# tgialoimtr/cnn_lstm_ctc_ocr

Hardware: AMD Instinct MI355X
Metric: line-crops/sec (train step) at 32x256 bs=256; CER vs ref (higher is better)
Workload: dtype bf16

## Files before the change

### cnn_lstm_ctc_ocr_amd/_lib.py

```python
import ctypes
import os

import torch

_HERE = os.path.dirname(os.path.abspath(__file__))
LIB_PATH = os.environ.get("OCRK_LIB") or os.path.join(_HERE, "libocrk.so")

OCRK_OK = 0
OCRK_ERR_INVALID_ARG = 1
OCRK_ERR_HIP = 2
OCRK_ERR_INFEASIBLE = 3

F32 = 0
BF16 = 1

_p = ctypes.c_void_p
_i32 = ctypes.c_int
_u32 = ctypes.c_uint
_i64 = ctypes.c_int64
_f32 = ctypes.c_float
_sz = ctypes.c_size_t

SIGNATURES = {
    "ocrk_version": [],
# ... 5 lines not shown
    "ocrk_set_f32_gemm_mode": [_i32],
    "ocrk_f32_gemm_exact": [],
    "ocrk_ctc_workspace_size": [_i32, _i32, _i32],
    "ocrk_ctc_loss": [_p, _p, _p, _p, _i32, _i32, _i32, _i32, _f32, _p, _p, _p, _p, _p, _sz, _p],
    "ocrk_ctc_greedy_decode": [_p, _p, _i32, _i32, _i32, _i32, _p, _p, _p, _p],
    "ocrk_ctc_beam_workspace_size": [_i32, _i32, _i32],
    "ocrk_gru_fwd_step": [_p, _p, _p, _p, _p, _p, _i32, _i32, _i32, _i32, _p, _p, _p, _p, _i32, _p],
    "ocrk_gru_fwd": [_p, _p, _p, _p, _p, _p, _i32, _i32, _i32, _p, _p, _p, _p, _i32, _p],
    "ocrk_gru_bwd": [_p, _p, _p, _p, _p, _p, _p, _i32, _i32, _i32, _p, _p, _p, _p, _i32, _p],
    "ocrk_ctc_beam_decode": [_p, _p, _i32, _i32, _i32, _i32, _i32, _i32, _p, _p, _p, _p, _sz, _p],
    "ocrk_crc32c": [_p, _sz, ctypes.c_uint32],
    "ocrk_edit_distance": [_p, _p, _i32, _p, _p, _i32, _i32, _p, _p, _p],
    "ocrk_conv1_fwd": [_p, _i32, _i32, _i32, _i32, _p, _p, _i32, _p, _i32, _p],
    "ocrk_conv1_wgrad_workspace_size": [_i32, _i32, _i32, _i32],
    "ocrk_conv1_bwd_weight": [_p, _i32, _p, _i32, _i32, _i32, _i32, _p, _p, _i32, _p, _sz, _i32, _p],
    "ocrk_conv2_bwd_data_conv1_wgrad_supported": [_i32, _i32, _i32, _i32, _i32, _i32],
    "ocrk_conv2_bwd_data_conv1_wgrad_workspace_size": [_i32, _i32, _i32],
    "ocrk_conv2_bwd_data_conv1_wgrad": [_p, _i32, _i32, _i32, _p, _p, _p, _p, _i32, _p, _p, _i32, _p, _sz, _i32,
                                        _p],
    "ocrk_conv12_bwd_supported": [_i32, _i32, _i32, _i32],
    "ocrk_conv12_bwd_workspace_size": [_i32, _i32, _i32],
    "ocrk_conv12_bwd": [_p, _i32, _i32, _i32, _p, _p, _p, _p, _i32, _p, _p, _p, _p, _p, _i32, _p, _sz, _i32, _p],
    "ocrk_conv12_fwd_supported": [_i32, _i32, _i32, _i32],
    "ocrk_conv12_fwd": [_p, _i32, _i32, _i32, _i32, _p, _p, _p, _p, _p, _p, _p, _p, _i32, _p],
    "ocrk_conv1_fwd_relu_bits": [_p, _i32, _i32, _i32, _i32, _p, _p, _i32, _p, _p, _i32, _p],
    "ocrk_conv_stats_tiles": [_i64],
    "ocrk_conv3x3_fwd": [_p, _i32, _i32, _i32, _i32, _p, _p, _i32, _p, _i32, _i32, _p, _i32, _p],
    "ocrk_conv3x3_bwd_data_workspace_size": [_i32, _i32, _i32, _i32],
    "ocrk_conv3x3_bwd_data": [_p, _i32, _i32, _i32, _i32, _p, _i32, _p, _p, _p, _i32, _p, _sz, _i32, _p],
    "ocrk_conv3x3_fwd_relu_bits_supported": [_i32, _i32, _i32, _i32, _i32, _i32],
    "ocrk_conv3x3_fwd_relu_bits": [_p, _i32, _i32, _i32, _i32, _p, _p, _i32, _p, _p, _i32, _p],
    "ocrk_conv3x3_bwd_data_bits_supported": [_i32, _i32, _i32, _i32, _i32, _i32],
    "ocrk_conv3x3_bwd_data_bits": [_p, _i32, _i32, _i32, _i32, _p, _i32, _p, _p, _p, _i32, _p, _sz, _i32, _p],
    "ocrk_conv3x3_bwd_data_bits_slab": [_p, _i32, _i32, _i32, _i32, _p, _i32, _p, _p, _p, _i32, _p],
    "ocrk_conv3x3_bwd_data_slab": [_p, _i32, _i32, _i32, _i32, _p, _i32, _p, _p, _p, _i32, _p],
    "ocrk_conv3x3_wgrad_workspace_size": [_i32, _i32, _i32, _i32, _i32],
    "ocrk_conv3x3_bwd_weight": [_p, _p, _i32, _i32, _i32, _i32, _i32, _p, _i32, _p, _sz, _i32, _p],
    "ocrk_bn_finalize_workspace_size": [_i32, _i32],
    "ocrk_bn_finalize": [_p, _i32, _i64, _i32, _f32, _f32, _p, _p, _p, _p, _p, _sz, _p],
    "ocrk_bn_finalize_tiles": [_p, _i32, _i32, _i64, _i32, _f32, _f32, _p, _p, _p, _p, _p, _sz, _p],
    "ocrk_conv3x3_fwd_rowstats_supported": [_i32, _i32, _i32, _i32, _i32],
    "ocrk_conv3x3_fwd_rowstats": [_p, _i32, _i32, _i32, _i32, _p, _p, _i32, _p, _i32, _p, _p],
    "ocrk_bn_infer_params": [_p, _p, _i32, _f32, _p, _p, _p],
    "ocrk_bn_relu_pool_fwd": [_p, _i32, _i32, _i32, _i32, _p, _p, _p, _p, _i32, _i32, _i32, _i32,
                              _p, _i32, _i32, _p],
    "ocrk_bn_bwd_workspace_size": [_i32, _i32, _i32, _i32],
    "ocrk_bn_relu_pool_bwd": [_p, _p, _i32, _i32, _i32, _i32, _p, _p, _p, _p, _i32, _i32, _i32, _i32,
                              _i32, _p, _p, _p, _p, _i32, _p, _sz, _i32, _p],
    "ocrk_bn_moments": [_p, _i32, _i32, _i64, _i32, _p, _p, _sz, _p],
    "ocrk_bn_finalize_moments": [_p, _i32, _f32, _f32, _p, _p, _p, _p, _p],
    "ocrk_bn_bwd_pooled_bias_slab_rows": [_i32, _i32, _i32, _i32, _i32, _i32, _i32, _i32],
    "ocrk_bn_relu_pool_bwd_pooled": [_p, _p, _p, _i32, _i32, _i32, _i32, _p, _p, _p, _p, _i32, _i32, _i32, _i32,
                                     _i32, _p, _p, _p, _p, _i32, _p, _p, _sz, _i32, _p],
    "ocrk_bn_relu_pool_bwd_reduce": [_p, _p, _i32, _i32, _i32, _i32, _p, _p, _p, _p, _i32, _i32, _i32, _i32,
                                     _i32, _p, _p, _i32, _p, _p, _sz, _i32, _p],
    "ocrk_bn_relu_pool_bwd_apply": [_p, _p, _i32, _i32, _i32, _i32, _p, _p, _p, _p, _i32, _i32, _i32, _i32,
                                    _i32, _p, _p, _p, _p, _i32, _p, _p, _sz, _i32, _p],
    "ocrk_bn_bwd_bias_slab_rows": [_i32, _i32, _i32, _i32, _i32, _i32, _i32, _i32],
    "ocrk_bn_relu_pool_bwd_slab": [_p, _p, _i32, _i32, _i32, _i32, _p, _p, _p, _p, _i32, _i32, _i32, _i32,
                                   _i32, _p, _p, _p, _i32, _p, _p, _sz, _i32, _p],
    "ocrk_lstm_fwd_step": [_p, _p, _p, _p, _p, _p, _i32, _i32, _i32, _i32, _p, _p, _p, _p, _i32, _p],
    "ocrk_lstm_bwd_step": [_p, _p, _p, _p, _p, _i32, _i32, _i32, _i32, _p, _p, _p, _p, _i32, _p],
    "ocrk_copy_batch": [_p, _i32, _i64, _p],
    "ocrk_gru_fwd_persistent_supported": [_i32, _i32],
    "ocrk_gru_fwd_persistent_workspace_size": [_i32, _i32],
    "ocrk_gru_fwd_persistent": [_p, _p, _p, _p, _i32, _i32, _i32, _p, _p, _p, _p, _p, _p, _p, _sz, _p],
    "ocrk_gru_bwd_persistent_supported": [_i32, _i32],
    "ocrk_gru_bwd_persistent_workspace_size": [_i32, _i32],
    "ocrk_gru_bwd_persistent": [_p, _p, _p, _i32, _i32, _i32, _p, _p, _p, _p, _p, _p, _p, _p, _sz, _p],
    "ocrk_persistent_flags_size": [_i32, _i32],
    "ocrk_lstm_fwd_persistent_supported": [_i32, _i32],
    "ocrk_lstm_fwd_persistent_workspace_size": [_i32, _i32],
    "ocrk_lstm_fwd_persistent": [_p, _p, _p, _i32, _i32, _i32, _p, _p, _p, _p, _p, _p, _p, _sz, _p],
    "ocrk_lstm_fwd_persistent_f32_supported": [_i32, _i32],
    "ocrk_lstm_fwd_persistent_f32_workspace_size": [_i32, _i32],
    "ocrk_lstm_fwd_persistent_f32_flags_size": [_i32, _i32],
    "ocrk_lstm_fwd_persistent_f32": [_p, _p, _p, _i32, _i32, _i32, _p, _p, _p, _p, _p, _p, _p, _sz, _p],
    "ocrk_lstm_bwd_persistent_f32_supported": [_i32, _i32],
    "ocrk_lstm_bwd_persistent_f32_workspace_size": [_i32, _i32],
    "ocrk_lstm_bwd_persistent_f32": [_p, _p, _i32, _i32, _i32, _p, _p, _p, _p, _p, _p, _p, _p, _sz, _p],
    "ocrk_lstm_bwd_persistent_supported": [_i32, _i32],
    "ocrk_lstm_bwd_persistent_workspace_size": [_i32, _i32],
    "ocrk_lstm_bwd_persistent_slices": [_i32, _i32],
    "ocrk_lstm_bwd_persistent": [_p, _p, _i32, _i32, _i32, _p, _p, _p, _p, _p, _p, _p, _p, _sz, _p],
    "ocrk_lstm_fwd": [_p, _p, _p, _p, _p, _i32, _i32, _i32, _p, _p, _p, _p, _i32, _p],
    "ocrk_lstm_bwd": [_p, _p, _p, _p, _i32, _i32, _i32, _p, _p, _p, _p, _i32, _p],
    "ocrk_gemm_workspace_size": [_i32, _i32, _i32, _i32],
    "ocrk_gemm": [_i32, _i32, _i32, _i32, _i32, _f32, _p, _i64, _i64, _p, _i64, _i64, _p, _i64, _i64,
                  _i32, _p, _i32, _i32, _i32, _i32, _i32, _p, _sz, _p],
    "ocrk_adam": [_p, _p, _p, _p, _i64, _f32, _f32, _f32, _f32, _f32, _p],
    "ocrk_adam_ex": [_p, _p, _p, _p, _i64, _f32, _f32, _f32, _f32, _f32, _u32, _p],
    "ocrk_cast": [_p, _i32, _p, _i32, _i64, _p],
    "ocrk_split_bf16": [_p, _i64, _p, _p, _p],
    "ocrk_permute3": [_p, _i32, _i32, _i32, _i32, _p, _i32, _p],
    "ocrk_strided_copy": [_p, _i64, _i64, _i64, _i64, _p, _i32, _i64, _i64, _p],
    "ocrk_colsum_workspace_size": [_i64, _i32],
    "ocrk_colsum": [_p, _i64, _i32, _i32, _p, _i32, _p, _sz, _p],
    "ocrk_slab_sum_workspace_size": [_i32],
    "ocrk_slab_sum": [_p, _i32, _i32, _i32, _p, _i32, _p, _sz, _p],
    "ocrk_relu_mask": [_p, _p, _i64, _f32, _p, _i32, _p],
    "ocrk_mul_scalar": [_p, _i64, _p, _p],
    "ocrk_mean": [_p, _i32, _p, _p],
    "ocrk_seq_len": [_p, _i32, _p, _p],
    "ocrk_timer_create": [_p],
    "ocrk_timer_record": [_p, _p],
    "ocrk_timer_elapsed": [_p, _p, _p],
    "ocrk_timer_destroy": [_p],
}
_RESTYPE = {"ocrk_last_error": ctypes.c_char_p}
_RESTYPE.update({n: ctypes.c_size_t for n in SIGNATURES if n.endswith("_workspace_size")})
_RESTYPE["ocrk_conv_stats_tiles"] = ctypes.c_size_t
_RESTYPE["ocrk_persistent_flags_size"] = ctypes.c_size_t
_RESTYPE["ocrk_bn_bwd_bias_slab_rows"] = ctypes.c_size_t
_RESTYPE["ocrk_bn_bwd_pooled_bias_slab_rows"] = ctypes.c_size_t
_RESTYPE["ocrk_crc32c"] = ctypes.c_uint32


class OcrkError(RuntimeError):

    def __init__(self, status, message):
        super().__init__(message)
        self.status = status


class InvalidArgumentError(OcrkError):
    """Mirrors tf.errors.InvalidArgumentError (e.g. infeasible CTC labels)."""


class DeviceError(OcrkError):
    """A device-side wait gave up (persistent recurrent kernels): its outputs are invalid."""


STATUS_CTC_INFEASIBLE = 1 << 1
STATUS_CTC_BAD_LENGTH = 1 << 2
STATUS_CTC_BAD_LABEL = 1 << 3
STATUS_LSTM_FWD_TIMEOUT = 1 << 4
STATUS_LSTM_BWD_TIMEOUT = 1 << 5
STATUS_LSTM_CENSUS = 1 << 6
STATUS_CTC = STATUS_CTC_INFEASIBLE | STATUS_CTC_BAD_LENGTH | STATUS_CTC_BAD_LABEL
STATUS_LSTM = STATUS_LSTM_FWD_TIMEOUT | STATUS_LSTM_BWD_TIMEOUT | STATUS_LSTM_CENSUS

_STATUS_TEXT = {
    STATUS_CTC_INFEASIBLE: "ctc_loss: not enough time for the target transition sequence "
                           "(label + repeats > sequence_length)",
    STATUS_CTC_BAD_LENGTH: "ctc_loss: a label length is negative or exceeds the labels' width",
    STATUS_CTC_BAD_LABEL: "ctc_loss: a label value is outside [0, num_classes - 1)",
    STATUS_LSTM_FWD_TIMEOUT: "persistent recurrent forward: a hand-off wait gave up (co-residency lost)",
    STATUS_LSTM_BWD_TIMEOUT: "persistent recurrent backward: a hand-off wait gave up (co-residency lost)",
    STATUS_LSTM_CENSUS: "persistent recurrent launch: the placement census gave up",
}


ON_DEVICE_ERROR = []


def raise_for_status(word):
    word = int(word)
    if not word:
        return
    text = "; ".join(t for b, t in _STATUS_TEXT.items() if word & b)
    if word & STATUS_LSTM:
        for fn in ON_DEVICE_ERROR:
            fn()
        raise DeviceError(OCRK_ERR_HIP, f"device status 0x{word:x}: {text}")
    raise InvalidArgumentError(OCRK_ERR_INFEASIBLE, f"device status 0x{word:x}: {text}")


# ... 84 lines not shown
```

### cnn_lstm_ctc_ocr_amd/csrc/bn.hip

```cpp
#include <type_traits>

#include "common.h"
#include "reduce.h"

using ocrk::slab_sum;
using ocrk::SLAB_P;

constexpr int BN_PARTS = 256;
__global__ void __launch_bounds__(256)
bn_stats_partial_kernel(const float* __restrict__ stats, int tiles, int64_t M, int tile_rows, int C, int rpb,
                        double* __restrict__ part) {
    __shared__ double sacc[3 * 256];
    const int NC = 2 * C;
    const int lanes = NC <= 256 ? 256 / NC : 1;
    const int full = (int)(M / tile_rows);
    const double inv_full = 1.0 / (double)tile_rows;
    const int t0 = blockIdx.x * rpb, t1 = min(tiles, t0 + rpb);
    double a[2] = {0, 0}, q[2] = {0, 0};
    const int lr = NC <= 256 ? threadIdx.x / NC : 0;
    const int j0 = NC <= 256 ? threadIdx.x % NC : threadIdx.x;
#pragma unroll
    for (int h = 0; h < 2; ++h) {
        const int j = j0 + 256 * h;
        if (j >= NC || (h == 1 && NC <= 256)) continue;
// ... 417 lines not shown
                        if (arg == dh * KW + j) dr[j][dh][i] += gp[i];
            }
#pragma unroll
            for (int j = 0; j < SW; ++j) retire(x0 + j, zr[j], dr[j]);
            if (!more) break;
            widen<T, NCH>(gpn, gp);
#pragma unroll
            for (int j = 0; j + SW < KW; ++j)
#pragma unroll
                for (int dh = 0; dh < KH; ++dh)
#pragma unroll
                    for (int i = 0; i < NCH; ++i) { zr[j][dh][i] = zr[j + SW][dh][i]; dr[j][dh][i] = dr[j + SW][dh][i]; }
#pragma unroll
            for (int j = 0; j < SW; ++j)
#pragma unroll
                for (int dh = 0; dh < KH; ++dh) {
                    widen<T, NCH>(nz[j][dh], zr[KW - SW + j][dh]);
#pragma unroll
                    for (int i = 0; i < NCH; ++i) dr[KW - SW + j][dh][i] = 0.f;
                }
        }
        const int xl = (wb - 1) * SW;
#pragma unroll
        for (int j = SW; j < KW; ++j) retire(xl + j, zr[j], dr[j]);
        for (int x = max(xl + KW, own0); x < own1; ++x) {
            float zc[KH][NCH], dc[KH][NCH];
#pragma unroll
            for (int dh = 0; dh < KH; ++dh) {
                if constexpr (APPLY) {
                    load_n<T, NCH>(zrow + ((int64_t)dh * W + x) * C, zc[dh]);
                } else {
#pragma unroll
                    for (int i = 0; i < NCH; ++i) zc[dh][i] = 0.f;
                }
#pragma unroll
                for (int i = 0; i < NCH; ++i) dc[dh][i] = 0.f;
            }
            retire(x, zc, dc);
        }
    }
#pragma unroll
    for (int i = 0; i < NCH; ++i) { red[threadIdx.x][i] = s1[i]; red[threadIdx.x][NCH + i] = s2[i]; }
    __syncthreads();
    const int nout = (APPLY && !DG) ? C : 2 * C;
    for (int o = threadIdx.x; o < nout; o += 256) {
        int which = o / C, c = o % C, gg = c / NCH, ci = c % NCH;
        float s = 0.f;
        for (int q = gg; q < 256; q += G) s += red[q][which * NCH + ci];
        slab[(int64_t)blockIdx.x * nout + o] = s;
    }
}


template <typename T>
__global__ void __launch_bounds__(256)
bn_bwd_pooled_sums_kernel(const T* __restrict__ p, const T* __restrict__ dp, int64_t items, int C,
                          const float* __restrict__ gamma, const float* __restrict__ beta,
                          const float* __restrict__ mean, const float* __restrict__ invstd, const T* __restrict__ z,
                          int B, int H, int W, int kh, int kw, int sh, int sw, int time_major, int items_per_block,
                          float* __restrict__ slab) {
    __shared__ float red[256][17];
    const int G = C / 8;
    const int g = threadIdx.x % G, c0 = 8 * g;
    float rg[8], bt[8], s1[8], s2[8];
    bool from_z = false;
#pragma unroll
    for (int i = 0; i < 8; ++i) {
        const float ga = gamma[c0 + i], be = beta[c0 + i];
        const float cz = fabsf(mean[c0 + i]) * invstd[c0 + i];
        from_z |= !(fabsf(be) <= fmaxf(4.f, cz) * fabsf(ga));
        rg[i] = ga != 0.f ? 1.f / ga : 0.f;
        bt[i] = be;
        s1[i] = s2[i] = 0.f;
    }
    const int64_t i0 = (int64_t)blockIdx.x * items_per_block;
    const int64_t i1 = min(items, i0 + items_per_block);
    if (from_z) {
        const int Ho = (H - kh) / sh + 1, Wo = (W - kw) / sw + 1;
        float sc[8], sf[8], mu[8], is[8];
#pragma unroll
        for (int i = 0; i < 8; ++i) {
            is[i] = invstd[c0 + i];
            mu[i] = mean[c0 + i];
            sc[i] = gamma[c0 + i] * is[i];
            sf[i] = beta[c0 + i] - mu[i] * sc[i];
        }
        for (int64_t it = i0 + threadIdx.x; it < i1; it += 256) {
            const int64_t pix = it / G;
            int b, ho, wo;
            if (time_major) {
                ho = (int)(pix % Ho);
                const int64_t r = pix / Ho;
                b = (int)(r % B);
                wo = (int)(r / B);
            } else {
                wo = (int)(pix % Wo);
                const int64_t r = pix / Wo;
                ho = (int)(r % Ho);
                b = (int)(r / Ho);
            }
            float best[8], zb[8];
#pragma unroll
            for (int i = 0; i < 8; ++i) { best[i] = -INFINITY; zb[i] = 0.f; }
            for (int dh = 0; dh < kh; ++dh)
                for (int dw = 0; dw < kw; ++dw) {
                    const F8 v = load8(z + (((int64_t)b * H + ho * sh + dh) * W + wo * sw + dw) * C + c0);
#pragma unroll
                    for (int i = 0; i < 8; ++i) {
                        const float y = fmaxf(fmaf(v.v[i], sc[i], sf[i]), 0.f);
                        if (y > best[i]) { best[i] = y; zb[i] = v.v[i]; }
                    }
                }
            const F8 dv = load8(dp + it * 8);
#pragma unroll
            for (int i = 0; i < 8; ++i) {
                const float d = best[i] > 0.f ? dv.v[i] : 0.f;
                s1[i] += d;
                s2[i] += d * ((zb[i] - mu[i]) * is[i]);
            }
        }
    } else {
        constexpr int U = 4;
        for (int64_t it = i0 + threadIdx.x; it < i1; it += 256 * U) {
            Pend8<T> pr[U], dr[U];
#pragma unroll
            for (int u = 0; u < U; ++u) {
                const int64_t q = min(it + 256 * u, i1 - 1);
                pr[u] = load_pend8(p + q * 8);
                dr[u] = load_pend8(dp + q * 8);
            }
#pragma unroll
            for (int u = 0; u < U; ++u) {
                if (it + 256 * u >= i1) break;
                const F8 pv = cvt8(pr[u]), dv = cvt8(dr[u]);
#pragma unroll
                for (int i = 0; i < 8; ++i) {
                    const float d = pv.v[i] > 0.f ? dv.v[i] : 0.f;
                    s1[i] += d;
                    s2[i] += d * ((pv.v[i] - bt[i]) * rg[i]);
                }
            }
        }
    }
#pragma unroll
    for (int i = 0; i < 8; ++i) { red[threadIdx.x][i] = s1[i]; red[threadIdx.x][8 + i] = s2[i]; }
    __syncthreads();
    for (int o = threadIdx.x; o < 2 * C; o += 256) {
        const int which = o / C, c = o % C, gg = c / 8, ci = c % 8;
        float s = 0.f;
        for (int q = gg; q < 256; q += G) s += red[q][which * 8 + ci];
        slab[(int64_t)blockIdx.x * 2 * C + o] = s;
    }
}

template <typename T>
__global__ void __launch_bounds__(256)
bn_bwd_apply_kernel(const T* __restrict__ z, const T* __restrict__ da_in, int npix, int C,
                    const float* __restrict__ mean, const float* __restrict__ invstd,
                    const float* __restrict__ gamma, const float* __restrict__ dsum, int items_per_block,
                    T* __restrict__ dz, float* __restrict__ bslab) {
    __shared__ float red[256][9];
    const int G = C / 8;
    const int items = npix * G;
    const int g = threadIdx.x % G, c0 = g * 8;
    const float inv_n = 1.f / (float)npix;
    float sc[8], mu[8], is[8], a[8], bb[8], cs[8];
#pragma unroll
    for (int i = 0; i < 8; ++i) {
        const int c = c0 + i;
        is[i] = invstd[c];
        mu[i] = mean[c];
        sc[i] = gamma[c] * is[i];
        a[i] = dsum[c] * inv_n;
        bb[i] = dsum[C + c] * inv_n;
        cs[i] = 0.f;
    }
    const int i0 = blockIdx.x * items_per_block;
    const int i1 = min(items, i0 + items_per_block);
    for (int it = i0 + threadIdx.x; it < i1; it += 256) {
        const int64_t off = (int64_t)(it / G) * C + c0;
        const F8 zz = load8(z + off), dd = load8(da_in + off);
        F8 out;
#pragma unroll
        for (int i = 0; i < 8; ++i) {
            const float xhat = (zz.v[i] - mu[i]) * is[i];
            out.v[i] = sc[i] * (dd.v[i] - a[i] - xhat * bb[i]);
            cs[i] += out.v[i];
        }
        store8(dz + off, out);
    }
    if (!bslab) return;
#pragma unroll
    for (int i = 0; i < 8; ++i) red[threadIdx.x][i] = cs[i];
    __syncthreads();
    for (int c = threadIdx.x; c < C; c += 256) {
        const int gg = c / 8, ci = c % 8;
        float s = 0.f;
        for (int q = gg; q < 256; q += G) s += red[q][ci];
        bslab[(int64_t)blockIdx.x * C + c] = s;
    }
}
// ... 121 lines not shown
    if (kh == 2 && kw == 2 && sw == 2) return 1;
    if (kh == 2 && kw == 2 && sw == 1) return 2;
    if (kh == 3 && kw == 1 && sw == 1) return 3;
    return 0;
}

static size_t bn_ws_floats(int64_t nb, int C) {
    size_t f = (size_t)SLAB_P * 2 * C * 2 + (size_t)(nb * 2 * C + 2 * C + nb * 2 * C);
    return (f + 3) / 4 * 4;
}

extern "C" size_t ocrk_bn_bwd_workspace_size(int B, int H, int W, int C) {
    int64_t items = (int64_t)B * H * W * (C / 8);
    int64_t nb = bn_bwd_blocks(items);
    nb = ocrk::cdiv(items, bn_bwd_ipb(items, nb));
    return bn_ws_floats(nb, C) * sizeof(float) + (size_t)B * H * W * C * sizeof(float);
}

struct WalkGrid { int nseg, tpb, blocks; };
static WalkGrid walk_grid(int B, int H, int W, int C, int kh, int kw, int sw, int64_t nb) {
    const int Ho = (H - kh) / kh + 1, Wo = (W - kw) / sw + 1;
    const int nseg = (int)ocrk::cdiv(Wo, bn_route_seg());
    const int64_t tasks = (int64_t)B * Ho * nseg * (C / bn_route_nch());
    const int64_t nbr = std::max<int64_t>(1, std::min<int64_t>(nb, ocrk::cdiv(tasks, 256)));
    const int64_t tpb = ocrk::cdiv(ocrk::cdiv(tasks, nbr), 256) * 256;
    return WalkGrid{nseg, (int)tpb, (int)ocrk::cdiv(tasks, tpb)};
}

static int64_t bn_bwd_bias_rows(int B, int H, int W, int C, int kh, int kw, int sh, int sw, bool pooled = false) {
    const int64_t items = (int64_t)B * H * W * (C / 8);
    int64_t nb = bn_bwd_blocks(items);
    nb = ocrk::cdiv(items, bn_bwd_ipb(items, nb));
    const int rk = bn_route_variant(kh, kw, sh, sw, H, W);
    if (rk == 1 || rk == 3 || (rk == 2 && pooled)) return walk_grid(B, H, W, C, kh, kw, sw, nb).blocks;
    return nb;
}

extern "C" size_t ocrk_bn_bwd_bias_slab_rows(int B, int H, int W, int C, int kh, int kw, int sh, int sw) {
    if (C < 8 || C % 8 != 0 || (int64_t)B * H * W == 0) return 1;
    return (size_t)bn_bwd_bias_rows(B, H, W, C, kh, kw, sh, sw);
}

extern "C" size_t ocrk_bn_bwd_pooled_bias_slab_rows(int B, int H, int W, int C, int kh, int kw, int sh, int sw) {
    if (!bn_route_variant(kh, kw, sh, sw, H, W)) return 0;
    if (C < 8 || C % 8 != 0 || (int64_t)B * H * W == 0) return 1;
    return (size_t)bn_bwd_bias_rows(B, H, W, C, kh, kw, sh, sw, true);
}

static int bn_bwd_impl(const void* z, const void* dp, int B, int H, int W, int C, const float* mean,
                       const float* invstd, const float* gamma, const float* beta, int kh, int kw, int sh, int sw,
                       int dp_time_major, void* dz, float* dgamma, float* dbeta, float* dbias, int accumulate,
                       float* bias_slab_out, void* ws, size_t ws_bytes, int dtype, void* stream, int phase = 0,
                       float* dsum_out = nullptr, const float* dsum_in = nullptr, const double* count = nullptr,
                       const void* pooled = nullptr) {
    OCRK_REQUIRE(C % 8 == 0 && 256 % (C / 8) == 0, "ocrk_bn_relu_pool_bwd: C=%d unsupported", C);
    OCRK_REQUIRE(ws_bytes >= ocrk_bn_bwd_workspace_size(B, H, W, C), "ocrk_bn_relu_pool_bwd: workspace too small");
    const int64_t items = (int64_t)B * H * W * (C / 8);
    OCRK_REQUIRE(items < (1ll << 31) && (int64_t)B * H * W < (1ll << 31), "ocrk_bn_relu_pool_bwd: tensor too large");
    if (items == 0) return OCRK_OK;
    int64_t nb = bn_bwd_blocks(items);
    const int64_t ipb = bn_bwd_ipb(items, nb);
    nb = ocrk::cdiv(items, ipb);
    double* part = (double*)ws;
    float* slab = (float*)(part + (size_t)SLAB_P * 2 * C);
    float* dsum = slab + nb * 2 * C;
    float* bslab = bias_slab_out ? bias_slab_out : dsum + 2 * C;
    void* da = (float*)ws + bn_ws_floats(nb, C);
    const int npix = B * H * W;
    hipStream_t s = ocrk::as_stream(stream);
    int nr = (int)nb;
    const int rk = bn_route_variant(kh, kw, sh, sw, H, W);
    const int seg = bn_route_seg();
    const bool from_pooled = pooled && rk;
    const int64_t pitems = from_pooled ? (int64_t)B * ((H - kh) / sh + 1) * ((W - kw) / sw + 1) * (C / 8) : 0;
    if (from_pooled) {
        nr = (int)std::max<int64_t>(1, std::min<int64_t>(nb, ocrk::cdiv(pitems, 256 * 4)));
    } else if (rk) {
        const int Ho = (H - kh) / kh + 1, Wo = (W - kw) / sw + 1;
        const int64_t tasks = (int64_t)B * Ho * ocrk::cdiv(Wo, seg) * (C / bn_route_nch());
        const int64_t nbr = std::min<int64_t>(nb, ocrk::cdiv(tasks, 256));
        nr = (int)ocrk::cdiv(tasks, ocrk::cdiv(ocrk::cdiv(tasks, nbr), 256) * 256);
    }
    int st = OCRK_OK;
    if (phase == 2) {
        bn_dsum_scale_kernel<<<ocrk::cdiv(2 * C, 256), 256, 0, s>>>(dsum_in, count, npix, 2 * C, dsum);
        st = ocrk::launch_status("ocrk_bn_relu_pool_bwd_apply scale");
        if (st) return st;
    } else if (from_pooled) {
        const int ipb2 = (int)(ocrk::cdiv(ocrk::cdiv(pitems, nr), 256) * 256);
        nr = (int)ocrk::cdiv(pitems, ipb2);
        if (dtype == OCRK_BF16)
            bn_bwd_pooled_sums_kernel<bf16><<<nr, 256, 0, s>>>((const bf16*)pooled, (const bf16*)dp, pitems, C, gamma,
                                                               beta, mean, invstd, (const bf16*)z, B, H, W, kh, kw,
                                                               sh, sw, dp_time_major, ipb2, slab);
        else
            bn_bwd_pooled_sums_kernel<float><<<nr, 256, 0, s>>>((const float*)pooled, (const float*)dp, pitems, C,
                                                                gamma, beta, mean, invstd, (const float*)z, B, H, W,
                                                                kh, kw, sh, sw, dp_time_major, ipb2, slab);
    } else if (rk) {
        const int Ho = (H - kh) / kh + 1, Wo = (W - kw) / sw + 1;
        const int nseg = (int)ocrk::cdiv(Wo, seg);
        const int64_t tasks = (int64_t)B * Ho * nseg * (C / bn_route_nch());
        const int64_t nbr = std::min<int64_t>(nb, ocrk::cdiv(tasks, 256));
        const int tpb = (int)(ocrk::cdiv(ocrk::cdiv(tasks, nbr), 256) * 256);
#define ROUTE_ARGS B, H, W, C, mean, invstd, gamma, beta, dp_time_major, nseg, tpb, slab
        if (dtype == OCRK_BF16) {
            const bf16 *zz = (const bf16*)z, *pp = (const bf16*)dp;
            bf16* dd = (bf16*)da;
            if (rk == 1) launch_route<bf16, 2, 2, 2, false>(seg, nr, s, zz, pp, ROUTE_ARGS, (bf16*)nullptr, (const float*)nullptr);
            else if (rk == 2) launch_route<bf16, 2, 2, 1, false>(seg, nr, s, zz, pp, ROUTE_ARGS, dd, (const float*)nullptr);
            else launch_route<bf16, 3, 1, 1, false>(seg, nr, s, zz, pp, ROUTE_ARGS, (bf16*)nullptr, (const float*)nullptr);
        } else {
            const float *zz = (const float*)z, *pp = (const float*)dp;
            float* dd = (float*)da;
            if (rk == 1) launch_route<float, 2, 2, 2, false>(seg, nr, s, zz, pp, ROUTE_ARGS, (float*)nullptr, (const float*)nullptr);
            else if (rk == 2) launch_route<float, 2, 2, 1, false>(seg, nr, s, zz, pp, ROUTE_ARGS, dd, (const float*)nullptr);
            else launch_route<float, 3, 1, 1, false>(seg, nr, s, zz, pp, ROUTE_ARGS, (float*)nullptr, (const float*)nullptr);
        }
#undef ROUTE_ARGS
    } else if (dtype == OCRK_BF16) {
        bn_bwd_reduce_kernel<bf16><<<nb, 256, 0, s>>>((const bf16*)z, (const bf16*)dp, B, H, W, C, mean, invstd, gamma, beta, kh, kw, sh, sw, dp_time_major, (int)ipb, slab, (bf16*)da);
    } else {
        bn_bwd_reduce_kernel<float><<<nb, 256, 0, s>>>((const float*)z, (const float*)dp, B, H, W, C, mean, invstd, gamma, beta, kh, kw, sh, sw, dp_time_major, (int)ipb, slab, (float*)da);
    }
    if (phase != 2) {
        st = ocrk::launch_status("ocrk_bn_relu_pool_bwd reduce");
        if (st) return st;
        st = slab_sum(slab, nr, 2 * C, part, phase == 1 ? dsum_out : dsum, dbeta, from_pooled ? nullptr : dgamma, C,
                      accumulate, s);
        if (st || phase == 1) return st;
    }
    if (rk == 1 || rk == 3 || (rk == 2 && from_pooled)) {
        const WalkGrid wg = walk_grid(B, H, W, C, kh, kw, sw, nb);
        const int nseg = wg.nseg, tpb = wg.tpb;
        nr = wg.blocks;
#define APPLY_ARGS B, H, W, C, mean, invstd, gamma, beta, dp_time_major, nseg, tpb, bslab
        const bool dg = from_pooled;
        if (dtype == OCRK_BF16) {
            const bf16 *zz = (const bf16*)z, *pp = (const bf16*)dp;
            bf16* dd = (bf16*)dz;
            const float* ds = dsum;
            if (rk == 1) launch_apply<bf16, 2, 2, 2>(dg, seg, nr, s, zz, pp, APPLY_ARGS, dd, ds);
            else if (rk == 2) launch_apply<bf16, 2, 2, 1>(dg, seg, nr, s, zz, pp, APPLY_ARGS, dd, ds);
            else launch_apply<bf16, 3, 1, 1>(dg, seg, nr, s, zz, pp, APPLY_ARGS, dd, ds);
        } else {
            const float *zz = (const float*)z, *pp = (const float*)dp;
            float* dd = (float*)dz;
            const float* ds = dsum;
            if (rk == 1) launch_apply<float, 2, 2, 2>(dg, seg, nr, s, zz, pp, APPLY_ARGS, dd, ds);
            else if (rk == 2) launch_apply<float, 2, 2, 1>(dg, seg, nr, s, zz, pp, APPLY_ARGS, dd, ds);
            else launch_apply<float, 3, 1, 1>(dg, seg, nr, s, zz, pp, APPLY_ARGS, dd, ds);
        }
#undef APPLY_ARGS
        st = ocrk::launch_status("ocrk_bn_relu_pool_bwd apply (window walk)");
        if (st || bias_slab_out) return st;
        if (dg) return slab_sum(bslab, nr, 2 * C, part, nullptr, dbias, dgamma, C, accumulate, s);
        if (!dbias) return st;
        return slab_sum(bslab, nr, C, part, nullptr, dbias, nullptr, C, accumulate, s);
    }
    float* bs = (dbias || bias_slab_out) ? bslab : nullptr;
    if (dtype == OCRK_BF16)
        bn_bwd_apply_kernel<bf16><<<nb, 256, 0, s>>>((const bf16*)z, (const bf16*)da, npix, C, mean, invstd, gamma, dsum, (int)ipb, (bf16*)dz, bs);
    else
        bn_bwd_apply_kernel<float><<<nb, 256, 0, s>>>((const float*)z, (const float*)da, npix, C, mean, invstd, gamma, dsum, (int)ipb, (float*)dz, bs);
    st = ocrk::launch_status("ocrk_bn_relu_pool_bwd apply");
    if (st || !dbias || bias_slab_out) return st;
    return slab_sum(bslab, (int)nb, C, part, nullptr, dbias, nullptr, C, accumulate, s);
}

extern "C" int ocrk_bn_relu_pool_bwd(const void* z, const void* dp, int B, int H, int W, int C,
                                     const float* mean, const float* invstd, const float* gamma,
                                     const float* beta, int kh, int kw, int sh, int sw, int dp_time_major,
                                     void* dz, float* dgamma, float* dbeta, float* dbias, int accumulate,
                                     void* ws, size_t ws_bytes, int dtype, void* stream) {
    return bn_bwd_impl(z, dp, B, H, W, C, mean, invstd, gamma, beta, kh, kw, sh, sw, dp_time_major, dz, dgamma,
                       dbeta, dbias, accumulate, nullptr, ws, ws_bytes, dtype, stream);
}

extern "C" int ocrk_bn_relu_pool_bwd_slab(const void* z, const void* dp, int B, int H, int W, int C,
                                          const float* mean, const float* invstd, const float* gamma,
                                          const float* beta, int kh, int kw, int sh, int sw, int dp_time_major,
                                          void* dz, float* dgamma, float* dbeta, int accumulate, float* bias_slab,
                                          void* ws, size_t ws_bytes, int dtype, void* stream) {
    OCRK_REQUIRE(bias_slab, "ocrk_bn_relu_pool_bwd_slab: bias_slab is required");
    return bn_bwd_impl(z, dp, B, H, W, C, mean, invstd, gamma, beta, kh, kw, sh, sw, dp_time_major, dz, dgamma,
                       dbeta, nullptr, accumulate, bias_slab, ws, ws_bytes, dtype, stream);
}

extern "C" int ocrk_bn_relu_pool_bwd_pooled(const void* z, const void* pooled, const void* dp, int B, int H, int W,
                                            int C, const float* mean, const float* invstd, const float* gamma,
                                            const float* beta, int kh, int kw, int sh, int sw, int dp_time_major,
                                            void* dz, float* dgamma, float* dbeta, float* dbias, int accumulate,
                                            float* bias_slab, void* ws, size_t ws_bytes, int dtype, void* stream) {
    OCRK_REQUIRE(pooled, "ocrk_bn_relu_pool_bwd_pooled: pooled is required");
    OCRK_REQUIRE(!bias_slab || bn_route_variant(kh, kw, sh, sw, H, W),
                 "ocrk_bn_relu_pool_bwd_pooled: bias_slab given but the pooled form is off for this pool "
                 "(ocrk_bn_bwd_pooled_bias_slab_rows() == 0)");
    return bn_bwd_impl(z, dp, B, H, W, C, mean, invstd, gamma, beta, kh, kw, sh, sw, dp_time_major, dz, dgamma,
                       dbeta, bias_slab ? nullptr : dbias, accumulate, bias_slab, ws, ws_bytes, dtype, stream, 0,
                       nullptr, nullptr, nullptr, pooled);
}

extern "C" int ocrk_bn_relu_pool_bwd_reduce(const void* z, const void* dp, int B, int H, int W, int C,
                                            const float* mean, const float* invstd, const float* gamma,
                                            const float* beta, int kh, int kw, int sh, int sw, int dp_time_major,
                                            float* dgamma, float* dbeta, int accumulate, float* dsum, void* ws,
                                            size_t ws_bytes, int dtype, void* stream) {
    OCRK_REQUIRE(dsum, "ocrk_bn_relu_pool_bwd_reduce: dsum is required");
    return bn_bwd_impl(z, dp, B, H, W, C, mean, invstd, gamma, beta, kh, kw, sh, sw, dp_time_major, nullptr, dgamma,
                       dbeta, nullptr, accumulate, nullptr, ws, ws_bytes, dtype, stream, 1, dsum);
}

extern "C" int ocrk_bn_relu_pool_bwd_apply(const void* z, const void* dp, int B, int H, int W, int C,
                                           const float* mean, const float* invstd, const float* gamma,
                                           const float* beta, int kh, int kw, int sh, int sw, int dp_time_major,
                                           const float* dsum, const double* count, void* dz, float* dbias,
                                           int accumulate, float* bias_slab, void* ws, size_t ws_bytes, int dtype,
                                           void* stream) {
    OCRK_REQUIRE(dsum && count && dz, "ocrk_bn_relu_pool_bwd_apply: dsum, count and dz are required");
    return bn_bwd_impl(z, dp, B, H, W, C, mean, invstd, gamma, beta, kh, kw, sh, sw, dp_time_major, dz, nullptr,
                       nullptr, dbias, accumulate, bias_slab, ws, ws_bytes, dtype, stream, 2, nullptr, dsum, count);
}
```

### cnn_lstm_ctc_ocr_amd/csrc/conv.hip

```cpp
#include "common.h"
#include "gemm.h"
#include "reduce.h"
#include "mfma_util.h"

constexpr int C1_PX = 256;
constexpr int C1_WR = 8;

template <typename TIn>
__device__ __forceinline__ float conv1_in(TIn v) {
    if constexpr (sizeof(TIn) == 1) {
#pragma clang fp contract(off)
        return (float)v * (1.0f / 255.0f) - 0.5f;
    } else {
        return to_f32(v);
    }
}

template <typename TIn, int ROWS>
__device__ __forceinline__ void conv1_stage(const TIn* __restrict__ x, int H, int W, int b, int h0, int wo0,
                                            float (*sx)[C1_PX + 2]) {
    constexpr int N = ROWS * (C1_PX + 2), IT = (N + 255) / 256;
    TIn v[IT];
    bool ok[IT];
#pragma unroll
// ... 191 lines not shown
}

extern "C" int ocrk_conv1_fwd(const void* x, int x_is_u8, int B, int H, int W, const float* w,
                              const float* bias, int cout, void* y, int dtype, void* stream) {
    return conv1_fwd_run(x, x_is_u8, B, H, W, w, bias, cout, y, nullptr, dtype, stream);
}

extern "C" int ocrk_conv1_fwd_relu_bits(const void* x, int x_is_u8, int B, int H, int W, const float* w,
                                        const float* bias, int cout, void* y, void* relu_bits, int dtype,
                                        void* stream) {
    OCRK_REQUIRE(relu_bits, "ocrk_conv1_fwd_relu_bits: null mask");
    return conv1_fwd_run(x, x_is_u8, B, H, W, w, bias, cout, y, (uint8_t*)relu_bits, dtype, stream);
}

static int64_t conv1_blocks(int B, int H, int W) {
    return std::max<int64_t>(1, (int64_t)B * ocrk::cdiv(H - 2, C1_GR) * ocrk::cdiv(W - 2, C1_PX));
}

extern "C" size_t ocrk_conv1_wgrad_workspace_size(int B, int H, int W, int cout) {
    return ((size_t)conv1_blocks(B, H, W) * 10 * cout * sizeof(float) + 15) / 16 * 16 +
           (size_t)ocrk::SLAB_P * 10 * cout * sizeof(double);
}

extern "C" int ocrk_conv1_bwd_weight(const void* x, int x_is_u8, const void* dz, int B, int H, int W,
                                     int cout, float* dw, float* db, int accumulate, void* ws,
                                     size_t ws_bytes, int dtype, void* stream) {
    OCRK_REQUIRE(cout == 32, "ocrk_conv1_bwd_weight: Cout=%d unsupported", cout);
    OCRK_REQUIRE(ws_bytes >= ocrk_conv1_wgrad_workspace_size(B, H, W, cout), "ocrk_conv1_bwd_weight: workspace too small");
    OCRK_REQUIRE(B >= 1 && H >= 3 && W >= 3, "ocrk_conv1_bwd_weight: bad shape B=%d H=%d W=%d", B, H, W);
    const int64_t nb = conv1_blocks(B, H, W);
    OCRK_REQUIRE(nb < (1ll << 31), "ocrk_conv1_bwd_weight: too many rows");
    hipStream_t s = ocrk::as_stream(stream);
    float* slab = (float*)ws;
    if (x_is_u8) {
        if (dtype == OCRK_BF16) conv1_wgrad_partial<uint8_t, bf16, 32><<<nb, 256, 0, s>>>((const uint8_t*)x, (const bf16*)dz, B, H, W, slab);
        else conv1_wgrad_partial<uint8_t, float, 32><<<nb, 256, 0, s>>>((const uint8_t*)x, (const float*)dz, B, H, W, slab);
    } else {
        if (dtype == OCRK_BF16) conv1_wgrad_partial<bf16, bf16, 32><<<nb, 256, 0, s>>>((const bf16*)x, (const bf16*)dz, B, H, W, slab);
        else conv1_wgrad_partial<float, float, 32><<<nb, 256, 0, s>>>((const float*)x, (const float*)dz, B, H, W, slab);
    }
    int st = ocrk::launch_status("ocrk_conv1_bwd_weight");
    if (st) return st;
    double* part = (double*)((char*)ws + ((size_t)nb * 10 * cout * sizeof(float) + 15) / 16 * 16);
    return ocrk::slab_sum(slab, (int)nb, 10 * cout, part, nullptr, dw, db, 9 * cout, accumulate, s);
}

extern "C" size_t ocrk_conv_stats_tiles(int64_t M) { return (size_t)ocrk::cdiv(M, 128); }

namespace ocrk {
int conv_direct_fwd(const void* x, int B, int H, int W, int cin, const void* w_nk, const float* bias, int cout,
                    void* y, int relu, float* stats, hipStream_t s);
int conv_direct_bwd_data(const void* dy, int B, int H, int W, int cout, const void* w_bwd, int cin, void* dx,
                         const void* relu_mask, float* stats, hipStream_t s);
size_t conv_direct_wgrad_ws_bytes(int B, int H, int W, int cin, int cout);
int conv_direct_wgrad(const void* x, const void* dy, int B, int H, int W, int cin, int cout, float* dw,
                      int accumulate, void* ws, size_t ws_bytes, hipStream_t s);
size_t conv_rows_wgrad_ws_bytes(int B, int cin, int cout);
bool conv_rows_fwd_covers(int B, int H, int W, int cin, int cout);
int conv_rows_fwd(const void* x, int B, int H, int W, int cin, const void* w_nk, const float* bias, int cout, void* y,
                  int relu, float* stats, hipStream_t s);
int conv_rows_dgrad(const void* dy, int B, int H, int W, int cout, const void* w_bwd, int cin, void* dx,
                    const void* relu_mask, float* stats, hipStream_t s);
int conv_rows_wgrad(const void* x, const void* dy, int B, int H, int W, int cin, int cout, float* dw, int accumulate,
                    void* ws, size_t ws_bytes, hipStream_t s);
bool conv_rows_dgrad_c1_covers(int B, int H, int W, int cin, int cout);
bool conv_rows_fwd_bits_covers(int B, int H, int W, int cin, int cout);
bool conv12_fwd_covers(int B, int H, int W);
int conv12_fwd(const void* img, int x_is_u8, int B, int H, int W, const float* w1, const float* b1,
               const void* w_nk2, const float* b2, void* y1, void* bits, void* z, float* stats, hipStream_t s);
int conv_rows_wgrad_c1x(const void* img, int x_is_u8, const float* w1, const float* b1, const void* dy, int B, int H,
                        int W, float* dw, int accumulate, void* ws, size_t ws_bytes, hipStream_t s);
int conv_rows_fwd_bits(const void* x, int B, int H, int W, int cin, const void* w_nk, const float* bias, int cout,
                       void* y, void* bits, hipStream_t s);
bool conv_rows_dgrad_bits_covers(int B, int H, int W, int cin, int cout);
int conv_rows_dgrad_bits(const void* dy, int B, int H, int W, int cout, const void* w_bwd, int cin, void* dx,
                         const void* bits, float* stats, hipStream_t s);
bool gemm_nt_enabled();
bool nt_staged_enabled();
int64_t conv_rows_dgrad_c1_parts(int B);
int conv_rows_dgrad_c1(const void* dy, int B, int H, int W, const void* w_bwd, const void* relu_mask,
                       const void* relu_bits, const void* x, int x_is_u8, float* part, hipStream_t s);
int64_t conv_rows_bwd_w2_parts(int B);
int conv_rows_bwd_w2(const void* dy, int B, int H, int W, const void* w_bwd, const void* relu_mask,
                     const void* relu_bits, const void* x, int x_is_u8, const float* w1, const float* b1,
                     float* c1part, float* w2part, float* dw2, int accumulate, hipStream_t s);
}

extern "C" int ocrk_conv12_fwd_supported(int B, int IH, int IW, int dtype) {
    return dtype == OCRK_BF16 && IH >= 3 && IW >= 3 && ocrk::conv12_fwd_covers(B, IH - 2, IW - 2) ? 1 : 0;
}

extern "C" int ocrk_conv12_fwd(const void* x, int x_is_u8, int B, int IH, int IW, const float* w1, const float* b1,
                               const void* w_nk2, const float* b2, void* y1, void* relu_bits, void* z, float* stats,
                               int dtype, void* stream) {
    OCRK_REQUIRE(ocrk_conv12_fwd_supported(B, IH, IW, dtype), "ocrk_conv12_fwd: B=%d IH=%d IW=%d dtype=%d not covered",
                 B, IH, IW, dtype);
    OCRK_REQUIRE(x && w1 && b1 && w_nk2 && relu_bits && z && stats, "ocrk_conv12_fwd: null pointer");
    return ocrk::conv12_fwd(x, x_is_u8, B, IH - 2, IW - 2, w1, b1, w_nk2, b2, y1, relu_bits, z, stats,
                            ocrk::as_stream(stream));
}

#ifdef OCRK_EXPERIMENTS
extern "C" int ocrk_conv2_bwd_weight_c1x_supported(int B, int IH, int IW, int dtype) {
    return ocrk_conv12_fwd_supported(B, IH, IW, dtype);
}

// ... 166 lines not shown
}

extern "C" size_t ocrk_conv3x3_bwd_data_workspace_size(int B, int H, int W, int cin) {
    return ((size_t)bwd_data_tiles(B, H, W) * 2 * cin * sizeof(float) + 7) / 8 * 8 +
           (size_t)ocrk::SLAB_P * cin * sizeof(double);
}

extern "C" int ocrk_conv3x3_bwd_data_bits(const void* dy, int B, int H, int W, int cout, const void* w_bwd, int cin,
                                          void* dx, const void* relu_bits, float* dbias, int accumulate, void* ws,
                                          size_t ws_bytes, int dtype, void* stream) {
    OCRK_REQUIRE(relu_bits && ocrk_conv3x3_bwd_data_bits_supported(B, H, W, cout, cin, dtype),
                 "ocrk_conv3x3_bwd_data_bits: B=%d H=%d W=%d %d<-%d dtype=%d not covered", B, H, W, cin, cout, dtype);
    hipStream_t s = ocrk::as_stream(stream);
    if (!dbias) return bwd_data_run(dy, B, H, W, cout, w_bwd, cin, dx, nullptr, nullptr, dtype, s, relu_bits);
    OCRK_REQUIRE(ws && ws_bytes >= ocrk_conv3x3_bwd_data_workspace_size(B, H, W, cin),
                 "ocrk_conv3x3_bwd_data_bits: workspace too small for the bias gradient");
    int st = bwd_data_run(dy, B, H, W, cout, w_bwd, cin, dx, nullptr, (float*)ws, dtype, s, relu_bits);
    if (st) return st;
    const int tiles = (int)bwd_data_tiles(B, H, W);
    double* part = (double*)((char*)ws + ((size_t)tiles * 2 * cin * sizeof(float) + 7) / 8 * 8);
    return ocrk::slab_sum((const float*)ws, tiles, cin, part, nullptr, dbias, nullptr, cin, accumulate, s, 2 * cin);
}

extern "C" int ocrk_conv3x3_bwd_data(const void* dy, int B, int H, int W, int cout, const void* w_bwd,
                                     int cin, void* dx, const void* relu_mask, float* dbias, int accumulate,
                                     void* ws, size_t ws_bytes, int dtype, void* stream) {
    hipStream_t s = ocrk::as_stream(stream);
    if (!dbias) return bwd_data_run(dy, B, H, W, cout, w_bwd, cin, dx, relu_mask, nullptr, dtype, s);
    OCRK_REQUIRE(ws && ws_bytes >= ocrk_conv3x3_bwd_data_workspace_size(B, H, W, cin),
                 "ocrk_conv3x3_bwd_data: workspace too small for the bias gradient");
    int st = bwd_data_run(dy, B, H, W, cout, w_bwd, cin, dx, relu_mask, (float*)ws, dtype, s);
    if (st) return st;
    const int tiles = (int)bwd_data_tiles(B, H, W);
    double* part = (double*)((char*)ws + ((size_t)tiles * 2 * cin * sizeof(float) + 7) / 8 * 8);
    return ocrk::slab_sum((const float*)ws, tiles, cin, part, nullptr, dbias, nullptr, cin, accumulate, s, 2 * cin);
}

extern "C" int ocrk_conv3x3_bwd_data_bits_slab(const void* dy, int B, int H, int W, int cout, const void* w_bwd,
                                               int cin, void* dx, const void* relu_bits, float* slab, int dtype,
                                               void* stream) {
    OCRK_REQUIRE(slab && relu_bits && ocrk_conv3x3_bwd_data_bits_supported(B, H, W, cout, cin, dtype),
                 "ocrk_conv3x3_bwd_data_bits_slab: B=%d H=%d W=%d %d<-%d dtype=%d not covered (or no slab)", B, H, W,
                 cin, cout, dtype);
    return bwd_data_run(dy, B, H, W, cout, w_bwd, cin, dx, nullptr, slab, dtype, ocrk::as_stream(stream), relu_bits);
}

extern "C" int ocrk_conv3x3_bwd_data_slab(const void* dy, int B, int H, int W, int cout, const void* w_bwd,
                                          int cin, void* dx, const void* relu_mask, float* slab, int dtype,
                                          void* stream) {
    OCRK_REQUIRE(slab, "ocrk_conv3x3_bwd_data_slab: slab is required");
    return bwd_data_run(dy, B, H, W, cout, w_bwd, cin, dx, relu_mask, slab, dtype, ocrk::as_stream(stream));
}

static int conv_tn_items() {
    const int64_t v = ocrk::opt(ocrk::OPT_CONV_TN_ITEMS);
    return v >= 16 ? (int)v : 192;
}

static int wgrad_splits(int64_t M, int cin, int cout) {
    if (ocrk::gemm_pptn_covers(ocrk::A_IM2COL_T, 9 * cin, cout, cin)) {
        const int64_t tiles = ocrk::cdiv(9 * cin, 256) * ocrk::cdiv(cout, 256);
        return (int)std::max<int64_t>(1, std::min<int64_t>(conv_tn_items() / tiles, M / 2048));
    }
    int64_t tiles = ocrk::cdiv(9 * cin, 128) * ocrk::cdiv(cout, cout <= 32 ? 32 : (cout <= 64 ? 64 : 128));
    const int64_t iv = ocrk::opt(ocrk::OPT_CONV_TN4_ITEMS);
    const int items = iv >= 16 ? (int)iv : 512;
    int64_t want = ocrk::cdiv(items, tiles);
    int64_t maxs = std::max<int64_t>(1, M / 4096);
    return (int)std::max<int64_t>(1, std::min<int64_t>(want, maxs));
}

extern "C" size_t ocrk_conv3x3_wgrad_workspace_size(int B, int H, int W, int cin, int cout) {
    int64_t M = (int64_t)B * H * W;
    size_t ws = std::max(ocrk::gemm_splitk_ws_bytes(9 * cin, cout, 1, wgrad_splits(M, cin, cout)),
                         ocrk::conv_direct_wgrad_ws_bytes(B, H, W, cin, cout));
    if ((cin == 32 && cout == 32) || (cout == 64 && (cin == 32 || cin == 64)) ||
        (cout == 128 && (cin == 64 || cin == 128)) || (cout == 256 && (cin == 128 || cin == 256)))
        ws = std::max(ws, ocrk::conv_rows_wgrad_ws_bytes(B, cin, cout));
    return ws;
}

extern "C" int ocrk_conv3x3_bwd_weight(const void* x, const void* dy, int B, int H, int W, int cin,
                                       int cout, float* dw, int accumulate, void* ws, size_t ws_bytes,
                                       int dtype, void* stream) {
    int64_t M = (int64_t)B * H * W;
    ocrk::GemmParams p = {};
    p.M = 9 * cin; p.N = cout; p.K = (int)M; p.batch = 1;
    p.A = x; p.B = dy; p.ldb = cout;
    p.C = dw; p.ldc = cout; p.c_bf16 = 0; p.accumulate = accumulate; p.alpha = 1.f;
    int splits = wgrad_splits(M, cin, cout);
    p.k_chunk = (int)(ocrk::cdiv(ocrk::cdiv(M, splits), 32) * 32);
    p.splits = (int)ocrk::cdiv(M, p.k_chunk);
    p.splitk_ws = (float*)ws;
    OCRK_REQUIRE(p.splits == 1 || ws_bytes >= ocrk::gemm_splitk_ws_bytes(p.M, p.N, 1, p.splits),
                 "ocrk_conv3x3_bwd_weight: workspace too small");
    p.convH = H; p.convW = W; p.convC = cin;
    if (dtype == OCRK_BF16) {
        int st = ocrk::conv_rows_wgrad(x, dy, B, H, W, cin, cout, dw, accumulate, ws, ws_bytes, ocrk::as_stream(stream));
        if (st >= 0) return st;
        st = ocrk::conv_direct_wgrad(x, dy, B, H, W, cin, cout, dw, accumulate, ws, ws_bytes, ocrk::as_stream(stream));
        if (st >= 0) return st;
    }
    return ocrk::gemm(p, ocrk::A_IM2COL_T, ocrk::B_KN, dtype, ocrk::as_stream(stream));
}
```

### cnn_lstm_ctc_ocr_amd/csrc/conv_direct.hip

```cpp
#include <climits>

#include "common.h"
#include "gemm.h"
#include "mfma_util.h"

namespace ocrk {

namespace {

constexpr int CM = 128;
constexpr unsigned DOOB = 0x80000000u;

__device__ __forceinline__ unsigned short bf16_u16(float v) { return __builtin_bit_cast(unsigned short, (bf16)v); }

__device__ __forceinline__ float row_sum16(float v) {
    v += __builtin_bit_cast(float, __builtin_amdgcn_mov_dpp(__builtin_bit_cast(int, v), 0x128, 0xf, 0xf, false));
    v += __builtin_bit_cast(float, __builtin_amdgcn_mov_dpp(__builtin_bit_cast(int, v), 0x124, 0xf, 0xf, false));
    v += __builtin_bit_cast(float, __builtin_amdgcn_mov_dpp(__builtin_bit_cast(int, v), 0x122, 0xf, 0xf, false));
    v += __builtin_bit_cast(float, __builtin_amdgcn_mov_dpp(__builtin_bit_cast(int, v), 0x121, 0xf, 0xf, false));
    return v;
}

__device__ __forceinline__ void dma16(__amdgpu_buffer_rsrc_t r, void* lds, unsigned voff) {
    __builtin_amdgcn_raw_ptr_buffer_load_lds(r, (__attribute__((address_space(3))) void*)lds, 16, voff, 0, 0, 0);
// ... 455 lines not shown
        return stats ? launch_direct<CI, NO, WN, false, true, false>(xb, wb, bias, nullptr, yb, stats, relu, B, H, W, s) \
                     : launch_direct<CI, NO, WN, false, false, false>(xb, wb, bias, nullptr, yb, nullptr, relu, B, H, W, s);
    OCRK_DF(32, 32, 1)
    OCRK_DF(32, 64, 1)
    OCRK_DF(64, 64, 2)
    OCRK_DF(64, 128, 4)
#undef OCRK_DF
    return -1;
}

size_t conv_direct_wgrad_ws_bytes(int B, int H, int W, int cin, int cout) {
    if (cin != 32 || (cout != 32 && cout != 64)) return 0;
    int dev = 0, ncu = 0;
    (void)hipGetDevice(&dev);
    (void)hipDeviceGetAttribute(&ncu, hipDeviceAttributeMultiprocessorCount, dev);
    const int per_cu = cout == 32 ? WgCfg<32>::PER_CU : WgCfg<64>::PER_CU;
    return (size_t)per_cu * (ncu > 0 ? ncu : 256) * 9 * cin * cout * sizeof(float);
}

int conv_direct_wgrad(const void* x, const void* dy, int B, int H, int W, int cin, int cout, float* dw,
                      int accumulate, void* ws, size_t ws_bytes, hipStream_t s) {
    const int mode = conv_direct_mode();
    if (mode == 0 || cin != 32 || (cout != 32 && cout != 64)) return -1;
    if (mode == 1 && cout != 32) return -1;
    if ((int64_t)B * H * W * (cout > cin ? cout : cin) * 2 > 0x7fffffffLL) return -1;
    if (ws_bytes < conv_direct_wgrad_ws_bytes(B, H, W, cin, cout) || (uintptr_t)ws % 16 != 0) return -1;
    const int M = B * H * W;
    const int nchunks = (int)cdiv(M, CM);
    int dev = 0, ncu = 0;
    (void)hipGetDevice(&dev);
    (void)hipDeviceGetAttribute(&ncu, hipDeviceAttributeMultiprocessorCount, dev);
    int grid = (cout == 32 ? WgCfg<32>::PER_CU : WgCfg<64>::PER_CU) * ncu;
    if (grid > nchunks) grid = nchunks;
    const int cpw = (int)cdiv(nchunks, grid);
    grid = (int)cdiv(nchunks, cpw);
    if (cout == 32) {
        static DeviceOnce cfg;
        set_dyn_lds(cfg, reinterpret_cast<const void*>(&conv3x3_wgrad_direct_kernel<32>), WgCfg<32>::LDS);
        conv3x3_wgrad_direct_kernel<32><<<grid, 256, WgCfg<32>::LDS, s>>>((const bf16*)x, (const bf16*)dy, (float*)ws, M, H, W, nchunks, cpw);
    } else {
        static DeviceOnce cfg;
        set_dyn_lds(cfg, reinterpret_cast<const void*>(&conv3x3_wgrad_direct_kernel<64>), WgCfg<64>::LDS);
        conv3x3_wgrad_direct_kernel<64><<<grid, 256, WgCfg<64>::LDS, s>>>((const bf16*)x, (const bf16*)dy, (float*)ws, M, H, W, nchunks, cpw);
    }
    int st = launch_status("conv3x3_wgrad_direct");
    if (st) return st;
    GemmParams p = {};
    p.M = 9 * cin; p.N = cout; p.K = M; p.batch = 1;
    p.C = dw; p.ldc = cout; p.c_bf16 = 0; p.accumulate = accumulate; p.alpha = 1.f;
    p.splits = grid; p.splitk_ws = (float*)ws;
    return splitk_finish(p, s);
}

int conv_direct_bwd_data(const void* dy, int B, int H, int W, int cout, const void* w_bwd, int cin, void* dx,
                         const void* relu_mask, float* stats, hipStream_t s) {
    const int mode = conv_direct_mode();
    if (mode == 0 || (int64_t)B * H * W * (cin > cout ? cin : cout) * 2 > 0x7fffffffLL) return -1;
    if (mode == 1 && cin != 32) return -1;
    const bf16* a = (const bf16*)dy;
    const bf16* wb = (const bf16*)w_bwd;
    const bf16* mk = (const bf16*)relu_mask;
    bf16* o = (bf16*)dx;
#define OCRK_DB(CI, NO, WN)                                                                                   \
    if (cout == CI && cin == NO) {                                                                          \
        if (mk) return stats ? launch_direct<CI, NO, WN, true, true, true>(a, wb, nullptr, mk, o, stats, 0, B, H, W, s)   \
                             : launch_direct<CI, NO, WN, true, false, true>(a, wb, nullptr, mk, o, nullptr, 0, B, H, W, s); \
        return stats ? launch_direct<CI, NO, WN, true, true, false>(a, wb, nullptr, nullptr, o, stats, 0, B, H, W, s)     \
                     : launch_direct<CI, NO, WN, true, false, false>(a, wb, nullptr, nullptr, o, nullptr, 0, B, H, W, s); \
    }
    OCRK_DB(32, 32, 1)
    OCRK_DB(64, 32, 1)
    OCRK_DB(64, 64, 2)
#undef OCRK_DB
    return -1;
}

}
```

### cnn_lstm_ctc_ocr_amd/csrc/gemm.h

```cpp
#pragma once
#include "common.h"

namespace ocrk {

enum AMode { A_ROWK = 0, A_COLK = 1, A_IM2COL = 2, A_IM2COL_FLIP = 3, A_IM2COL_T = 4 };
enum BMode { B_NK = 0, B_KN = 1 };

struct GemmParams {
    int M, N, K;
    int batch;
    const void* A; int64_t lda; int64_t strideA;
    const void* B; int64_t ldb; int64_t strideB;
    void* C; int64_t ldc; int64_t strideC;
    int c_bf16;
    const float* bias; int64_t strideBias;
    const void* mask; int64_t ldmask;
    int accumulate;
    int relu;
    float alpha;
    float* stats;
    float* splitk_ws;
    int splits;
    int k_chunk;
    int convH, convW, convC;
    int epi_staged;
    const void* mask_bits;
    void* relu_bits;
};

struct TileIdx { int bm, bn; bool valid; };
__device__ __forceinline__ TileIdx xcd_tile(int tm, int tn) {
    const int nT = tm * tn, per = (nT + 7) >> 3;
    const int t = (int)(blockIdx.x & 7) * per + (int)(blockIdx.x >> 3);
    if (t >= nT) return {0, 0, false};
    constexpr int GM = 4;
    const int gsz = GM * tn, grp = t / gsz, first = grp * GM;
    const int gm = min(GM, tm - first), w = t - grp * gsz;
    return {first + w % gm, w / gm, true};
}
__host__ __forceinline__ unsigned xcd_grid(int tm, int tn) { return 8u * (unsigned)((tm * tn + 7) / 8); }

int gemm(const GemmParams& p, int amode, int bmode, int dtype, hipStream_t stream);

size_t gemm_splitk_ws_bytes(int M, int N, int batch, int splits);
int splitk_finish(const GemmParams& p, hipStream_t stream);

int gemm_nt(const GemmParams& p, int amode, int bmode, int dtype, hipStream_t stream);
bool f32_exact_mfma();

int gemm_pp(const GemmParams& p, int amode, int bmode, int dtype, hipStream_t stream);

bool gemm_pptn_covers(int amode, int M, int N, int convC);
int gemm_pptn(const GemmParams& p, int amode, int bmode, int dtype, hipStream_t stream);

int gemm_tn(const GemmParams& p, int amode, int bmode, int dtype, hipStream_t stream);

}
```

### cnn_lstm_ctc_ocr_amd/csrc/gemm.hip

```cpp
#include <atomic>
#include <cstdlib>
#include <type_traits>

#include "gemm.h"
#include "mfma_util.h"

namespace ocrk {

template <int AM, typename CT>
__device__ __forceinline__ const CT* a_addr(const GemmParams& p, const CT* A, int m, int k, bool& ok) {
    if constexpr (AM == A_ROWK) {
        ok = m < p.M && k < p.K;
        return A + (int64_t)m * p.lda + k;
    } else if constexpr (AM == A_COLK) {
        ok = m < p.M && k < p.K;
        return A + (int64_t)k * p.lda + m;
    } else {
        int pix, kidx;
        if constexpr (AM == A_IM2COL_T) { pix = k; kidx = m; ok = k < p.K && m < p.M; }
        else { pix = m; kidx = k; ok = m < p.M && k < p.K; }
        const int C = p.convC, W = p.convW, H = p.convH;
        int tap = kidx / C, c = kidx - tap * C;
        int kh = tap / 3, kw = tap - kh * 3;
        int w = pix % W, t2 = pix / W, h = t2 % H, b = t2 / H;
// ... 476 lines not shown
static std::atomic<int> g_f32_mode{0};

bool f32_exact_mfma() {
    return opt(OPT_F32_MFMA) == 1 || g_f32_mode.load(std::memory_order_relaxed) == 1;
}

template <typename CT, int AM, int BMD>
static int launch_tiles(const GemmParams& p0, hipStream_t stream) {
    GemmParams p = p0;
    int TBM = 128, TBN = p.N <= 32 ? 32 : (p.N <= 64 ? 64 : 128);
    dim3 grid((unsigned)cdiv(p.M, TBM), (unsigned)cdiv(p.N, TBN), (unsigned)(p.batch * p.splits));
    constexpr bool F32 = sizeof(CT) == 4;
    if (F32 && !f32_exact_mfma()) {
        if (TBN == 32) gemm_kernel<CT, AM, BMD, 128, 32, F32><<<grid, 256, 0, stream>>>(p);
        else if (TBN == 64) gemm_kernel<CT, AM, BMD, 128, 64, F32><<<grid, 256, 0, stream>>>(p);
        else gemm_kernel<CT, AM, BMD, 128, 128, F32><<<grid, 256, 0, stream>>>(p);
    } else if (TBN == 32) gemm_kernel<CT, AM, BMD, 128, 32><<<grid, 256, 0, stream>>>(p);
    else if (TBN == 64) gemm_kernel<CT, AM, BMD, 128, 64><<<grid, 256, 0, stream>>>(p);
    else gemm_kernel<CT, AM, BMD, 128, 128><<<grid, 256, 0, stream>>>(p);
    int st = launch_status("gemm");
    if (st != OCRK_OK) return st;
    return splitk_finish(p, stream);
}

template <typename CT>
static int dispatch_modes(const GemmParams& p, int amode, int bmode, hipStream_t s) {
#define GM(AMx, BMx) if (amode == AMx && bmode == BMx) return launch_tiles<CT, AMx, BMx>(p, s)
    GM(A_ROWK, B_NK);
    GM(A_ROWK, B_KN);
    GM(A_COLK, B_KN);
    GM(A_IM2COL, B_NK);
    GM(A_IM2COL_FLIP, B_NK);
    GM(A_IM2COL_T, B_KN);
#undef GM
    set_error("gemm: unsupported operand modes A=%d B=%d", amode, bmode);
    return OCRK_ERR_INVALID_ARG;
}

int gemm(const GemmParams& p, int amode, int bmode, int dtype, hipStream_t stream) {
    if (p.M <= 0 || p.N <= 0 || p.batch <= 0) return OCRK_OK;
    OCRK_REQUIRE(p.K >= 0 && p.splits >= 1 && p.k_chunk > 0 && p.k_chunk % 32 == 0,
                 "gemm: bad K=%d splits=%d k_chunk=%d", p.K, p.splits, p.k_chunk);
    bool a_rows = (amode == A_COLK || amode == A_IM2COL_T);
    OCRK_REQUIRE(p.K % 8 == 0 || (a_rows && bmode == B_KN),
                 "gemm: K=%d must be a multiple of 8 for k-contiguous operands", p.K);
    OCRK_REQUIRE(!a_rows || p.M % 8 == 0, "gemm: M=%d must be a multiple of 8 for this A mode", p.M);
    OCRK_REQUIRE(bmode != B_KN || p.N % 8 == 0, "gemm: N=%d must be a multiple of 8 for B_KN", p.N);
    OCRK_REQUIRE(amode < A_IM2COL || p.convC % 8 == 0, "gemm: conv channels must be a multiple of 8");
    OCRK_REQUIRE(!(p.stats && (p.splits > 1 || p.batch > 1)), "gemm: stats need splits=1, batch=1");
    OCRK_REQUIRE(!(p.accumulate && p.c_bf16), "gemm: accumulate needs an f32 C");
    if (p.mask_bits || p.relu_bits) {
        const int st = gemm_nt(p, amode, bmode, dtype, stream);
        OCRK_REQUIRE(st >= 0, "gemm: ReLU bit masks need the NT engine (bf16 C, staged epilogue) for this shape");
        return st;
    }
    int nt = gemm_pp(p, amode, bmode, dtype, stream);
    if (nt >= 0) return nt != OCRK_OK ? nt : splitk_finish(p, stream);
    nt = gemm_nt(p, amode, bmode, dtype, stream);
    if (nt < 0) nt = gemm_pptn(p, amode, bmode, dtype, stream);
    if (nt < 0) nt = gemm_tn(p, amode, bmode, dtype, stream);
    if (nt >= 0) return nt != OCRK_OK ? nt : splitk_finish(p, stream);
    if (dtype == OCRK_BF16) return dispatch_modes<bf16>(p, amode, bmode, stream);
    if (dtype == OCRK_F32) return dispatch_modes<float>(p, amode, bmode, stream);
    set_error("gemm: unsupported dtype %d", dtype);
    return OCRK_ERR_INVALID_ARG;
}

}

extern "C" int ocrk_set_f32_gemm_mode(int mode) {
    OCRK_REQUIRE(mode == 0 || mode == 1, "ocrk_set_f32_gemm_mode: mode %d not 0 (bf16x3) or 1 (exact)", mode);
    return ocrk::g_f32_mode.exchange(mode);
}

extern "C" int ocrk_f32_gemm_exact(void) { return ocrk::f32_exact_mfma() ? 1 : 0; }

extern "C" size_t ocrk_gemm_workspace_size(int M, int N, int batch, int splits) {
    return ocrk::gemm_splitk_ws_bytes(M, N, batch, splits);
}

extern "C" int ocrk_gemm(int trans_a, int trans_b, int M, int N, int K, float alpha, const void* A,
                         int64_t lda, int64_t stride_a, const void* B, int64_t ldb, int64_t stride_b,
                         void* C, int64_t ldc, int64_t stride_c, int c_dtype, const float* bias,
                         int relu, int accumulate, int batch, int dtype, int splits, void* ws,
                         size_t ws_bytes, void* stream) {
    ocrk::GemmParams p = {};
    p.M = M; p.N = N; p.K = K; p.batch = batch < 1 ? 1 : batch;
    p.A = A; p.lda = lda; p.strideA = stride_a;
    p.B = B; p.ldb = ldb; p.strideB = stride_b;
    p.C = C; p.ldc = ldc; p.strideC = stride_c;
    p.c_bf16 = c_dtype == OCRK_BF16;
    p.bias = bias; p.strideBias = 0;
    p.relu = relu; p.accumulate = accumulate; p.alpha = alpha;
    p.splits = splits < 1 ? 1 : splits;
    int kc = (int)ocrk::cdiv(K, p.splits);
    p.k_chunk = (int)ocrk::cdiv(kc < 32 ? 32 : kc, 32) * 32;
    p.splits = (int)ocrk::cdiv(K > 0 ? K : 1, p.k_chunk);
    p.splitk_ws = (float*)ws;
    OCRK_REQUIRE(p.splits == 1 || ws_bytes >= ocrk::gemm_splitk_ws_bytes(M, N, p.batch, p.splits),
                 "ocrk_gemm: split-K workspace too small");
    int amode = trans_a ? ocrk::A_COLK : ocrk::A_ROWK;
    int bmode = trans_b ? ocrk::B_NK : ocrk::B_KN;
    return ocrk::gemm(p, amode, bmode, dtype, ocrk::as_stream(stream));
}
```

### cnn_lstm_ctc_ocr_amd/csrc/gemm_nt.hip

```cpp
#include "gemm.h"
#include "mfma_util.h"

namespace ocrk {

namespace {

constexpr unsigned NT_OOB = 0x80000000u;

constexpr unsigned NT_BADROW = 0xFFFFFFFFu;

__device__ __forceinline__ void lds_dma16(__amdgpu_buffer_rsrc_t r, void* lds, unsigned voff) {
    __builtin_amdgcn_raw_ptr_buffer_load_lds(r, (__attribute__((address_space(3))) void*)lds, 16, voff, 0, 0, 0);
}

template <int BM, int BN, int BK, int S, int WAVES_M, int AM, int NW = 4, bool F32 = false, bool EXACT = false,
          bool X6 = false, bool TU = false>
__global__ void __launch_bounds__(NW * 64) gemm_nt_kernel(const GemmParams p) {
    constexpr bool ST = NW == 4;
    constexpr int WAVES_N = NW / WAVES_M;
    constexpr int WM = BM / WAVES_M, WN = BN / WAVES_N;
    constexpr int TM = WM / 16, TN = WN / 16;
    constexpr int ESZ = F32 ? 4 : 2;
    constexpr int EPC = 16 / ESZ;
    constexpr int ROWB = BK * ESZ;
    constexpr int RPI = 1024 / ROWB;
    constexpr int CPR = ROWB / 16;
    constexpr int A_BYTES = BM * ROWB, B_BYTES = BN * ROWB, STAGE = A_BYTES + B_BYTES;
    constexpr int NA = BM / (NW * RPI), NB = BN >= NW * RPI ? BN / (NW * RPI) : 1;
    constexpr int BBLK = BN / RPI;
    constexpr int NPS = NA + NB;
    static_assert((BK == 32 || BK == 64) && S >= 2, "BK 32 or 64, >= 2 stages");
    static_assert(!F32 || BK == 32, "fp32 operands: BK = 32 (128-B rows)");
    static_assert(BM % (NW * RPI) == 0 && BN % RPI == 0 && (BN < NW * RPI || BN % (NW * RPI) == 0), "tile");
    static_assert(TM >= 1 && TN >= 1, "wave tile");
    extern __shared__ __attribute__((aligned(16))) char smem[];

    const int tid = threadIdx.x, lane = tid & 63, wave = __builtin_amdgcn_readfirstlane(tid >> 6);
    const int wm = wave / WAVES_N, wn = wave % WAVES_N;
    const TileIdx tix = xcd_tile((p.M + BM - 1) / BM, (p.N + BN - 1) / BN);
    if (!tix.valid) return;
    const int m0 = tix.bm * BM, n0 = tix.bn * BN;
    const int zb = blockIdx.z / p.splits, zs = blockIdx.z - zb * p.splits;
    const char* A = reinterpret_cast<const char*>(p.A) + zb * p.strideA * ESZ;
    const char* B = reinterpret_cast<const char*>(p.B) + zb * p.strideB * ESZ;
    const int kbeg = zs * p.k_chunk;
    const int kend = min(p.K, kbeg + p.k_chunk);
    const int nk = max(0, (kend - kbeg + BK - 1) / BK);

    int64_t a_elems, b_elems = (int64_t)p.N * p.ldb;
    if constexpr (AM == A_ROWK) a_elems = (int64_t)p.M * p.lda;
    else a_elems = (int64_t)p.M * p.convC;
    const __amdgpu_buffer_rsrc_t ra = uniform_rsrc(A, a_elems * ESZ);
    const __amdgpu_buffer_rsrc_t rb = uniform_rsrc(B, b_elems * ESZ);

    const int lrow = lane / CPR;
    const int chunk = ROWB == 128 ? ((lane & 7) ^ lrow) : ((lane & 3) ^ ((lrow >> 2) & 3));

    unsigned aoff[NA], ahw[NA];
#pragma unroll
    for (int i = 0; i < NA; ++i) {
        const int m = m0 + (i * NW + wave) * RPI + lrow;
        ahw[i] = 0;
        if constexpr (AM == A_ROWK) {
            aoff[i] = m < p.M ? (unsigned)((int64_t)m * p.lda * ESZ) : NT_BADROW;
        } else {
            const int W = p.convW, H = p.convH;
            const int mm = m < p.M ? m : 0;
            const int w = mm % W, h = (mm / W) % H;
            ahw[i] = ((unsigned)h << 16) | (unsigned)w;
// ... 174 lines not shown
#pragma unroll
                for (int j = 0; j < TN; ++j)
#pragma unroll
                    for (int e = 0; e < 8; ++e)
                        acc[i][j] = __builtin_amdgcn_mfma_f32_16x16x4f32(av.e(e), bv[j].e(e), acc[i][j], 0, 0, 0);
            }
            continue;
        }
        if constexpr (F32) {
            const int s0 = ((2 * g) ^ swz) * 16, s1 = ((2 * g + 1) ^ swz) * 16;
            auto frag = [&](const char* row, bf16x8& hi, bf16x8& lo) {
                V8<float> v;
                v.q0 = *reinterpret_cast<const f32x4*>(row + s0);
                v.q1 = *reinterpret_cast<const f32x4*>(row + s1);
                u32x4 h, l;
                split8_bf16(v, h, l);
                hi = __builtin_bit_cast(bf16x8, h);
                lo = __builtin_bit_cast(bf16x8, l);
            };
            bf16x8 bh[TN], bl[TN];
#pragma unroll
            for (int j = 0; j < TN; ++j) frag(sb + (wn * WN + j * 16 + i16) * ROWB, bh[j], bl[j]);
#pragma unroll
            for (int i = 0; i < TM; ++i) {
                bf16x8 ah, al;
                frag(sa + (wm * WM + i * 16 + i16) * ROWB, ah, al);
#pragma unroll
                for (int j = 0; j < TN; ++j) {
                    acc[i][j] = __builtin_amdgcn_mfma_f32_16x16x32_bf16(al, bh[j], acc[i][j], 0, 0, 0);
                    acc[i][j] = __builtin_amdgcn_mfma_f32_16x16x32_bf16(ah, bl[j], acc[i][j], 0, 0, 0);
                    acc[i][j] = __builtin_amdgcn_mfma_f32_16x16x32_bf16(ah, bh[j], acc[i][j], 0, 0, 0);
                }
            }
            continue;
        }
#pragma unroll
        for (int kk = 0; kk < BK / 32; ++kk) {
            const int slot = ((kk * 4 + g) ^ swz) * 16;
            bf16x8 bfr[TN];
#pragma unroll
            for (int j = 0; j < TN; ++j)
                bfr[j] = *reinterpret_cast<const bf16x8*>(sb + (wn * WN + j * 16 + i16) * ROWB + slot);
#pragma unroll
            for (int i = 0; i < TM; ++i) {
                const bf16x8 af = *reinterpret_cast<const bf16x8*>(sa + (wm * WM + i * 16 + i16) * ROWB + slot);
#pragma unroll
                for (int j = 0; j < TN; ++j)
                    acc[i][j] = __builtin_amdgcn_mfma_f32_16x16x32_bf16(af, bfr[j], acc[i][j], 0, 0, 0);
            }
        }
    }
    __syncthreads();

    const int row_base = m0 + wm * WM + (lane >> 4) * 4;
    const int col_base = n0 + wn * WN + (lane & 15);
    if (p.splits > 1) {
        float* ws = p.splitk_ws + ((int64_t)zb * p.splits + zs) * (int64_t)p.M * p.N;
#pragma unroll
        for (int i = 0; i < TM; ++i)
#pragma unroll
            for (int j = 0; j < TN; ++j)
#pragma unroll
                for (int r = 0; r < 4; ++r) {
                    const int row = row_base + i * 16 + r, col = col_base + j * 16;
                    if (row < p.M && col < p.N) ws[(int64_t)row * p.N + col] = acc[i][j][r];
                }
        return;
    }
    const float* bias = p.bias ? p.bias + zb * p.strideBias : nullptr;
    const bf16* mask = reinterpret_cast<const bf16*>(p.mask);
    const float* maskf = reinterpret_cast<const float*>(p.mask);
    float* Cf = reinterpret_cast<float*>(p.C) + zb * p.strideC;
    bf16* Cb = reinterpret_cast<bf16*>(p.C) + zb * p.strideC;
    constexpr int TP = BN * 2 + 16, T_OFF = 4096, CPT = BN / 8;
    constexpr bool TILE_FITS = T_OFF + BM * TP <= S * STAGE;
    const bool staged = TILE_FITS && p.epi_staged;
    char* tile = smem + T_OFF;
    const uint8_t* mbits = reinterpret_cast<const uint8_t*>(p.mask_bits);
    if (staged && (mask || mbits)) {
        for (int q = tid; q < BM * CPT; q += NW * 64) {
            const int r = q / CPT, cc = q - r * CPT;
            const int row = m0 + r, col = n0 + 8 * cc;
            uint4 v = make_uint4(0u, 0u, 0u, 0u);
            if (row < p.M && col < p.N) {
                if (mbits) {
                    const unsigned m = mbits[(int64_t)row * (p.N >> 3) + (col >> 3)];
                    unsigned w[4];
#pragma unroll
                    for (int i = 0; i < 4; ++i)
                        w[i] = ((m >> (2 * i)) & 1u ? 0x3f80u : 0u) | ((m >> (2 * i + 1)) & 1u ? 0x3f800000u : 0u);
                    v = make_uint4(w[0], w[1], w[2], w[3]);
                } else {
                    v = *reinterpret_cast<const uint4*>(mask + (int64_t)row * p.ldmask + col);
                }
            }
            *reinterpret_cast<uint4*>(tile + r * TP + cc * 16) = v;
        }
        __syncthreads();
    }
#pragma unroll
    for (int j = 0; j < TN; ++j) {
        const int col = col_base + j * 16;
        const float bcol = (bias && col < p.N) ? bias[col] : 0.f;
#pragma unroll
        for (int i = 0; i < TM; ++i)
#pragma unroll
            for (int r = 0; r < 4; ++r) {
                const int row = row_base + i * 16 + r;
                float v = p.alpha * acc[i][j][r] + bcol;
                if (row < p.M && col < p.N) {
                    if (staged) {
                        bf16* e = reinterpret_cast<bf16*>(tile + (row - m0) * TP + (col - n0) * 2);
                        if ((mask || mbits) && !((float)*e > 0.f)) v = 0.f;
                        if (p.relu) v = fmaxf(v, 0.f);
                        *e = (bf16)v;
                    } else {
                        if constexpr (F32) {
                            if (maskf && !(maskf[(int64_t)row * p.ldmask + col] > 0.f)) v = 0.f;
                        } else {
                            if (mask && !((float)mask[(int64_t)row * p.ldmask + col] > 0.f)) v = 0.f;
                        }
                        if (p.relu) v = fmaxf(v, 0.f);
                        const int64_t off = (int64_t)row * p.ldc + col;
                        if (p.c_bf16) {
                            Cb[off] = (bf16)v;
                        } else {
                            if (p.accumulate) v += Cf[off];
                            Cf[off] = v;
                        }
                    }
                }
                acc[i][j][r] = v;
            }
    }
    if (staged) {
        __syncthreads();
        uint8_t* rbits = reinterpret_cast<uint8_t*>(p.relu_bits);
        for (int q = tid; q < BM * CPT; q += NW * 64) {
            const int r = q / CPT, cc = q - r * CPT;
            const int row = m0 + r, col = n0 + 8 * cc;
            if (row < p.M && col < p.N) {
                const uint4 v = *reinterpret_cast<const uint4*>(tile + r * TP + cc * 16);
                *reinterpret_cast<uint4*>(Cb + (int64_t)row * p.ldc + col) = v;
                if (rbits) {
                    const unsigned w[4] = {v.x, v.y, v.z, v.w};
                    unsigned m = 0;
#pragma unroll
                    for (int i = 0; i < 4; ++i) {
                        m |= (__uint_as_float(w[i] << 16) > 0.f ? 1u : 0u) << (2 * i);
                        m |= (__uint_as_float(w[i] & 0xffff0000u) > 0.f ? 1u : 0u) << (2 * i + 1);
                    }
                    rbits[(int64_t)row * (p.N >> 3) + (col >> 3)] = (uint8_t)m;
                }
            }
        }
    }
    if constexpr (!ST) return;
    if (!p.stats) return;

    float* s_red = reinterpret_cast<float*>(smem);
    const int valid_rows = min(BM, p.M - m0);
    float tsum[TN];
#pragma unroll
    for (int j = 0; j < TN; ++j) {
        float s = 0.f;
#pragma unroll
        for (int i = 0; i < TM; ++i)
#pragma unroll
            for (int r = 0; r < 4; ++r)
                if (row_base + i * 16 + r < p.M) s += acc[i][j][r];
        s = add_xor32(add_xor16(s));
        tsum[j] = s;
    }
    if (lane < 16)
#pragma unroll
        for (int j = 0; j < TN; ++j) s_red[wm * BN + wn * WN + j * 16 + lane] = tsum[j];
    __syncthreads();
    float tmean[TN];
#pragma unroll
    for (int j = 0; j < TN; ++j) {
        const int c = wn * WN + j * 16 + (lane & 15);
        float s = 0.f;
#pragma unroll
        for (int q = 0; q < WAVES_M; ++q) s += s_red[q * BN + c];
        tsum[j] = s;
        tmean[j] = s / (float)valid_rows;
    }
    __syncthreads();
#pragma unroll
    for (int j = 0; j < TN; ++j) {
        float s = 0.f;
#pragma unroll
        for (int i = 0; i < TM; ++i)
#pragma unroll
            for (int r = 0; r < 4; ++r)
                if (row_base + i * 16 + r < p.M) {
                    const float d = acc[i][j][r] - tmean[j];
                    s += d * d;
                }
        s = add_xor32(add_xor16(s));
        if (lane < 16) s_red[wm * BN + wn * WN + j * 16 + lane] = s;
    }
    __syncthreads();
    if (wm == 0 && lane < 16) {
#pragma unroll
        for (int j = 0; j < TN; ++j) {
            const int c = wn * WN + j * 16 + lane;
            if (n0 + c < p.N) {
                float m2 = 0.f;
#pragma unroll
                for (int q = 0; q < WAVES_M; ++q) m2 += s_red[q * BN + c];
                float* st = p.stats + (int64_t)tix.bm * 2 * p.N;
                st[n0 + c] = tsum[j];
                st[p.N + n0 + c] = m2;
            }
        }
    }
}

template <int BM, int BN, int BK, int S, int WAVES_M, int AM, int NW, bool F32, bool EXACT, bool X6, bool TU>
int launch_nt_k(const GemmParams& p, hipStream_t stream) {
    constexpr int LDS = S * (BM + BN) * BK * (F32 ? 4 : 2);
    static DeviceOnce configured;
    set_dyn_lds(configured,
                reinterpret_cast<const void*>(&gemm_nt_kernel<BM, BN, BK, S, WAVES_M, AM, NW, F32, EXACT, X6, TU>),
                LDS);
    dim3 grid(xcd_grid((int)cdiv(p.M, BM), (int)cdiv(p.N, BN)), 1u, (unsigned)(p.batch * p.splits));
    gemm_nt_kernel<BM, BN, BK, S, WAVES_M, AM, NW, F32, EXACT, X6, TU><<<grid, NW * 64, LDS, stream>>>(p);
    return launch_status("gemm_nt");
}

template <int BK, int AM>
bool nt_tap_uniform(const GemmParams& p) {
    return AM != A_ROWK && opt(OPT_NT_TAP_UNIFORM) != 0 && p.convC % BK == 0 &&
           (p.splits == 1 || p.k_chunk % BK == 0);
}

template <int BM, int BN, int BK, int S, int WAVES_M, int AM, int NW = 4, bool F32 = false, bool EXACT = false,
          bool X6 = false>
int launch_nt(const GemmParams& p, hipStream_t stream) {
    if constexpr (NW == 8 && !F32) {
        if (p.stats) return launch_nt<128, 128, 64, 2, 2, AM, 4>(p, stream);
    }
    if constexpr (AM != A_ROWK) {
        if (nt_tap_uniform<BK, AM>(p))
            return launch_nt_k<BM, BN, BK, S, WAVES_M, AM, NW, F32, EXACT, X6, true>(p, stream);
    }
    return launch_nt_k<BM, BN, BK, S, WAVES_M, AM, NW, F32, EXACT, X6, false>(p, stream);
}

template <int AM, bool EXACT = false, bool X6 = false>
int dispatch_nt_f32(const GemmParams& p, hipStream_t s) {
    if (p.N <= 32) return launch_nt<128, 32, 32, 3, 4, AM, 4, true, EXACT, X6>(p, s);
    if (p.N <= 64) return launch_nt<128, 64, 32, 3, 2, AM, 4, true, EXACT, X6>(p, s);
    return launch_nt<128, 128, 32, 2, 2, AM, 4, true, EXACT, X6>(p, s);
}

#ifdef OCRK_EXPERIMENTS
int nt_cfg() {
    static const int c = [] {
        const char* e = getenv("OCRK_GEMM_NT_CFG");
        return e ? atoi(e) : -1;
    }();
    return c;
}
#endif

template <int AM>
int dispatch_nt(const GemmParams& p, hipStream_t s) {
#ifdef OCRK_EXPERIMENTS
    switch (nt_cfg()) {
        case 0: return launch_nt<256, 128, 64, 3, 2, AM>(p, s);
        case 1: return launch_nt<128, 128, 64, 2, 2, AM>(p, s);
        case 2: return launch_nt<128, 128, 32, 3, 2, AM>(p, s);
        case 3: return launch_nt<128, 128, 64, 3, 2, AM>(p, s);
        case 4: return launch_nt<256, 128, 32, 4, 2, AM>(p, s);
        case 5: return launch_nt<128, 128, 32, 4, 2, AM>(p, s);
        case 6: return launch_nt<256, 256, 64, 2, 2, AM, 8>(p, s);
        case 7: return launch_nt<256, 128, 64, 2, 4, AM, 8>(p, s);
        case 8: return launch_nt<256, 256, 32, 3, 2, AM, 8>(p, s);
        case 9: return launch_nt<256, 256, 32, 4, 2, AM, 8>(p, s);
        case 10: return launch_nt<256, 128, 32, 4, 4, AM, 8>(p, s);
        case 11: return launch_nt<128, 128, 32, 6, 2, AM>(p, s);
        case 12: return launch_nt<128, 128, 32, 5, 2, AM>(p, s);
        case 13: return launch_nt<128, 128, 64, 4, 2, AM>(p, s);
        case 14: return launch_nt<128, 64, 64, 3, 2, AM>(p, s);
        case 15: return launch_nt<64, 96, 64, 3, 2, AM>(p, s);
        case 16: return launch_nt<64, 128, 32, 4, 2, AM>(p, s);
        case 17: return launch_nt<128, 96, 64, 3, 2, AM>(p, s);
        case 18: return launch_nt<64, 128, 64, 3, 2, AM>(p, s);
        default: break;
    }
#endif
    if (p.N <= 32) return launch_nt<128, 32, 32, 3, 4, AM>(p, s);
    if (p.N <= 64) return launch_nt<128, 64, 32, 3, 2, AM>(p, s);
    if (p.N <= 96) return launch_nt<64, 96, 64, 3, 2, AM>(p, s);
    if (p.N >= 512 && p.M >= 16384 && !p.mask_bits && !p.relu_bits) return launch_nt<256, 256, 64, 2, 2, AM, 8>(p, s);
    return launch_nt<128, 128, 64, 2, 2, AM>(p, s);
}

}

bool gemm_nt_enabled() {
    return opt(OPT_GEMM_NT) != 0;
}

bool nt_staged_enabled() {
    return opt(OPT_GEMM_NT_STAGED) != 0;
}

int gemm_nt(const GemmParams& p0, int amode, int bmode, int dtype, hipStream_t stream) {
    if (!gemm_nt_enabled() || bmode != B_NK) return -1;
    if (dtype == OCRK_F32) {
        const bool exact = f32_exact_mfma();
        if (exact && (amode == A_ROWK || !opt(OPT_NT_F32_EXACT))) return -1;
        if (p0.c_bf16 || (p0.mask && !opt(OPT_NT_F32_MASK)) || p0.K % 4 != 0 || (p0.k_chunk < 256 && p0.N > 64))
            return -1;
        GemmParams p = p0;
        p.epi_staged = 0;
        if (amode == A_ROWK) {
            if (p.lda % 4 != 0 || p.ldb % 4 != 0) return -1;
            return dispatch_nt_f32<A_ROWK>(p, stream);
        }
        if (p.convC % 4 != 0 || p.ldb % 4 != 0) return -1;
        const bool x6 = exact && opt(OPT_NT_F32_X6);
        if (amode == A_IM2COL) return x6 ? dispatch_nt_f32<A_IM2COL, true, true>(p, stream)
                                      : exact ? dispatch_nt_f32<A_IM2COL, true>(p, stream)
                                              : dispatch_nt_f32<A_IM2COL>(p, stream);
        if (amode == A_IM2COL_FLIP) return x6 ? dispatch_nt_f32<A_IM2COL_FLIP, true, true>(p, stream)
                                           : exact ? dispatch_nt_f32<A_IM2COL_FLIP, true>(p, stream)
                                                   : dispatch_nt_f32<A_IM2COL_FLIP>(p, stream);
        return -1;
    }
    if (dtype != OCRK_BF16) return -1;
    GemmParams p = p0;
    p.epi_staged = nt_staged_enabled() && p.c_bf16 && p.splits == 1 && p.N % 8 == 0 && p.ldc % 8 == 0 &&
                   p.strideC % 8 == 0 && (uintptr_t)p.C % 16 == 0 &&
                   (!p.mask || (p.ldmask % 8 == 0 && (uintptr_t)p.mask % 16 == 0));
    if (p.K % 8 != 0 || (p.k_chunk < 512 && p.N > 64)) return -1;
    if ((p.mask_bits || p.relu_bits) && (!p.epi_staged || p.batch != 1 || p.ldc != p.N)) return -1;
    if (amode == A_ROWK) {
        if (p.lda % 8 != 0 || p.ldb % 8 != 0) return -1;
        return dispatch_nt<A_ROWK>(p, stream);
    }
    if (amode == A_IM2COL) return dispatch_nt<A_IM2COL>(p, stream);
    if (amode == A_IM2COL_FLIP) return dispatch_nt<A_IM2COL_FLIP>(p, stream);
    return -1;
}

}
```

### cnn_lstm_ctc_ocr_amd/kernels.py

```python
import ctypes

import torch

from . import _lib, options
from ._lib import ptr, call

F32, BF16 = _lib.F32, _lib.BF16
_DT = {torch.float32: F32, torch.bfloat16: BF16}


def dtype_code(dt):
    try:
        return _DT[dt]
    except KeyError:
        raise TypeError(f"unsupported dtype {dt}; libocrk computes in float32 or bfloat16")


def _stream(t):
    return _lib.stream_ptr(t.device)


def _chk(*ts):
    for t in ts:
        if t is None:
# ... 143 lines not shown
         dtype_code(x.dtype), _stream(x))
    return y, bits


def conv3x3_fwd(x, w_nk, bias, relu, stats=None, y_dtype=None):
    _chk(x, w_nk, bias, stats)
    B, H, W, Cin = x.shape
    Cout = w_nk.shape[0]
    y_dtype = y_dtype or x.dtype
    y = torch.empty(B, H, W, Cout, dtype=y_dtype, device=x.device)
    call("ocrk_conv3x3_fwd", ptr(x), B, H, W, Cin, ptr(w_nk), ptr(bias), Cout, ptr(y), dtype_code(y_dtype),
         int(relu), ptr(stats), dtype_code(x.dtype), _stream(x))
    return y


def conv3x3_bwd_data(dy, w_bwd, relu_mask=None, dbias=None, accumulate=True, defer=None, relu_bits=None):
    _chk(dy, w_bwd, relu_mask, dbias, relu_bits)
    B, H, W, Cout = dy.shape
    Cin = w_bwd.shape[0]
    dx = torch.empty(B, H, W, Cin, dtype=dy.dtype, device=dy.device)
    if relu_bits is not None:
        if relu_mask is not None:
            raise ValueError("relu_bits replaces relu_mask")
        if dbias is not None and defer is not None:
            tiles = conv_stats_tiles(B * H * W)
            slab = torch.empty(tiles, 2 * Cin, dtype=torch.float32, device=dy.device)
            call("ocrk_conv3x3_bwd_data_bits_slab", ptr(dy), B, H, W, Cout, ptr(w_bwd), Cin, ptr(dx), ptr(relu_bits),
                 ptr(slab), dtype_code(dy.dtype), _stream(dy))
            defer.append((lambda: slab_sum(slab, tiles, Cin, 2 * Cin, dbias, accumulate), (slab,)))
            return dx
        nb, ws = 0, None
        if dbias is not None:
            nb = _lib.lib().ocrk_conv3x3_bwd_data_workspace_size(B, H, W, Cin)
            ws = _ws(nb, dy.device)
        call("ocrk_conv3x3_bwd_data_bits", ptr(dy), B, H, W, Cout, ptr(w_bwd), Cin, ptr(dx), ptr(relu_bits),
             ptr(dbias), int(accumulate), ptr(ws), nb, dtype_code(dy.dtype), _stream(dy))
        return dx
    if dbias is not None and defer is not None:
        tiles = conv_stats_tiles(B * H * W)
        slab = torch.empty(tiles, 2 * Cin, dtype=torch.float32, device=dy.device)
        call("ocrk_conv3x3_bwd_data_slab", ptr(dy), B, H, W, Cout, ptr(w_bwd), Cin, ptr(dx), ptr(relu_mask),
             ptr(slab), dtype_code(dy.dtype), _stream(dy))
        defer.append((lambda: slab_sum(slab, tiles, Cin, 2 * Cin, dbias, accumulate), (slab,)))
        return dx
    nb, ws = 0, None
    if dbias is not None:
        nb = _lib.lib().ocrk_conv3x3_bwd_data_workspace_size(B, H, W, Cin)
        ws = _ws(nb, dy.device)
    call("ocrk_conv3x3_bwd_data", ptr(dy), B, H, W, Cout, ptr(w_bwd), Cin, ptr(dx), ptr(relu_mask), ptr(dbias),
         int(accumulate), ptr(ws), nb, dtype_code(dy.dtype), _stream(dy))
    return dx


def conv3x3_bwd_weight(x, dy, dw, accumulate=True):
    _chk(x, dy, dw)
    B, H, W, Cin = x.shape
    Cout = dy.shape[-1]
    nb = _lib.lib().ocrk_conv3x3_wgrad_workspace_size(B, H, W, Cin, Cout)
    ws = _ws(nb, x.device)
    call("ocrk_conv3x3_bwd_weight", ptr(x), ptr(dy), B, H, W, Cin, Cout, ptr(dw), int(accumulate), ptr(ws), nb,
         dtype_code(x.dtype), _stream(x))


def bn_finalize(stats, M, C, eps, momentum, moving_mean=None, moving_var=None, tile_rows=128):
    _chk(stats, moving_mean, moving_var)
    tiles = stats.shape[0]
    mean = torch.empty(C, dtype=torch.float32, device=stats.device)
    invstd = torch.empty_like(mean)
    nb = _lib.lib().ocrk_bn_finalize_workspace_size(tiles, C)
    ws = _ws(nb, stats.device)
    call("ocrk_bn_finalize_tiles", ptr(stats), tiles, int(tile_rows), M, C, float(eps), float(momentum), ptr(mean),
         ptr(invstd), ptr(moving_mean), ptr(moving_var), ptr(ws), nb, _stream(stats))
    return mean, invstd


def bn_finalize_sync(stats, M, C, eps, momentum, moving_mean, moving_var, tile_rows, group):
    import torch.distributed as dist
    _chk(stats, moving_mean, moving_var)
    tiles = stats.shape[0]
    moments = torch.empty(3 * C + 1, dtype=torch.float64, device=stats.device)
    nb = _lib.lib().ocrk_bn_finalize_workspace_size(tiles, C)
    ws = _ws(nb, stats.device)
    call("ocrk_bn_moments", ptr(stats), tiles, int(tile_rows), M, C, ptr(moments), ptr(ws), nb, _stream(stats))
    dist.all_reduce(moments, op=dist.ReduceOp.SUM, group=group)
    mean = torch.empty(C, dtype=torch.float32, device=stats.device)
    invstd = torch.empty_like(mean)
    call("ocrk_bn_finalize_moments", ptr(moments), C, float(eps), float(momentum), ptr(mean), ptr(invstd),
         ptr(moving_mean), ptr(moving_var), _stream(stats))
    return mean, invstd, moments[3 * C:]


def conv3x3_fwd_rowstats_ok(x, cout):
    if x.dtype != torch.bfloat16 or not x.is_cuda:
        return False
    B, H, W, cin = x.shape
    return bool(_lib.lib().ocrk_conv3x3_fwd_rowstats_supported(B, H, W, cin, cout))


def conv3x3_fwd_rowstats(x, w_nk, bias, relu=False):
    _chk(x, w_nk, bias)
    B, H, W, cin = x.shape
    cout = w_nk.shape[0]
    y = torch.empty(B, H, W, cout, dtype=x.dtype, device=x.device)
    stats = torch.empty(B * H, 2, cout, dtype=torch.float32, device=x.device)
    call("ocrk_conv3x3_fwd_rowstats", ptr(x), B, H, W, cin, ptr(w_nk), ptr(bias), cout, ptr(y), int(relu),
         ptr(stats), _stream(x))
    return y, stats


def bn_infer_params(moving_mean, moving_var, eps):
    _chk(moving_mean, moving_var)
    C = moving_mean.numel()
    mean = torch.empty(C, dtype=torch.float32, device=moving_mean.device)
    invstd = torch.empty_like(mean)
    call("ocrk_bn_infer_params", ptr(moving_mean), ptr(moving_var), C, float(eps), ptr(mean), ptr(invstd),
         _stream(moving_mean))
    return mean, invstd


def bn_relu_pool_fwd(z, mean, invstd, gamma, beta, pool, time_major=False):
    _chk(z, mean, invstd, gamma, beta)
    B, H, W, C = z.shape
    kh, kw, sh, sw = pool
    Ho, Wo = (H - kh) // sh + 1, (W - kw) // sw + 1
    shape = (Wo, B, C) if time_major else (B, Ho, Wo, C)
    out = torch.empty(shape, dtype=z.dtype, device=z.device)
    call("ocrk_bn_relu_pool_fwd", ptr(z), B, H, W, C, ptr(mean), ptr(invstd), ptr(gamma), ptr(beta), kh, kw, sh, sw,
         ptr(out), int(time_major), dtype_code(z.dtype), _stream(z))
    return out


def bn_relu_pool_bwd(z, dp, mean, invstd, gamma, beta, pool, dp_time_major, dgamma, dbeta, accumulate=True,
                     dbias=None, defer=None, sync=None, pooled=None):
    _chk(z, dp, mean, invstd, gamma, beta, dgamma, dbeta, dbias, pooled)
    B, H, W, C = z.shape
    kh, kw, sh, sw = pool
    nb = _lib.lib().ocrk_bn_bwd_workspace_size(B, H, W, C)
    ws = _ws(nb, z.device)
    dz = torch.empty_like(z)
    if sync is not None:
        return _bn_bwd_sync(z, dp, mean, invstd, gamma, beta, pool, dp_time_major, dgamma, dbeta, accumulate, dbias,
                            defer, sync, dz, ws, nb)
    if pooled is not None:
        if pooled.shape != dp.shape or pooled.dtype != dp.dtype:
            raise ValueError("pooled must have dp's shape and dtype")
        rows = _lib.lib().ocrk_bn_bwd_pooled_bias_slab_rows(B, H, W, C, kh, kw, sh, sw)
        if rows == 0:
            pooled = None
    if pooled is not None:
        slab = None
        if dbias is not None and defer is not None:
            slab = torch.empty(rows, 2 * C, dtype=torch.float32, device=z.device)
        call("ocrk_bn_relu_pool_bwd_pooled", ptr(z), ptr(pooled), ptr(dp), B, H, W, C, ptr(mean), ptr(invstd),
             ptr(gamma), ptr(beta), kh, kw, sh, sw, int(dp_time_major), ptr(dz), ptr(dgamma), ptr(dbeta),
             ptr(dbias), int(accumulate), ptr(slab), ptr(ws), nb, dtype_code(z.dtype), _stream(z))
        if slab is not None:
            def _late():
                slab_sum(slab, rows, C, 2 * C, dbias, accumulate)
                slab_sum(slab.view(-1)[C:], rows, C, 2 * C, dgamma, accumulate)
            defer.append((_late, (slab,)))
        return dz
    if dbias is not None and defer is not None:
        rows = _lib.lib().ocrk_bn_bwd_bias_slab_rows(B, H, W, C, kh, kw, sh, sw)
        slab = torch.empty(rows, C, dtype=torch.float32, device=z.device)
        call("ocrk_bn_relu_pool_bwd_slab", ptr(z), ptr(dp), B, H, W, C, ptr(mean), ptr(invstd), ptr(gamma),
             ptr(beta), kh, kw, sh, sw, int(dp_time_major), ptr(dz), ptr(dgamma), ptr(dbeta), int(accumulate),
             ptr(slab), ptr(ws), nb, dtype_code(z.dtype), _stream(z))
        defer.append((lambda: slab_sum(slab, rows, C, C, dbias, accumulate), (slab,)))
        return dz
    call("ocrk_bn_relu_pool_bwd", ptr(z), ptr(dp), B, H, W, C, ptr(mean), ptr(invstd), ptr(gamma), ptr(beta),
         kh, kw, sh, sw, int(dp_time_major), ptr(dz), ptr(dgamma), ptr(dbeta), ptr(dbias), int(accumulate),
         ptr(ws), nb,
         dtype_code(z.dtype), _stream(z))
    return dz


def _bn_bwd_sync(z, dp, mean, invstd, gamma, beta, pool, dp_time_major, dgamma, dbeta, accumulate, dbias, defer,
                 sync, dz, ws, nb):
    import torch.distributed as dist
    group, count = sync
    B, H, W, C = z.shape
    kh, kw, sh, sw = pool
    dsum = torch.empty(2 * C, dtype=torch.float32, device=z.device)
    args = (ptr(z), ptr(dp), B, H, W, C, ptr(mean), ptr(invstd), ptr(gamma), ptr(beta), kh, kw, sh, sw,
            int(dp_time_major))
    call("ocrk_bn_relu_pool_bwd_reduce", *args, ptr(dgamma), ptr(dbeta), int(accumulate), ptr(dsum), ptr(ws), nb,
         dtype_code(z.dtype), _stream(z))
    dist.all_reduce(dsum, op=dist.ReduceOp.SUM, group=group)
    slab = None
    if dbias is not None and defer is not None:
        rows = _lib.lib().ocrk_bn_bwd_bias_slab_rows(B, H, W, C, kh, kw, sh, sw)
        slab = torch.empty(rows, C, dtype=torch.float32, device=z.device)
    call("ocrk_bn_relu_pool_bwd_apply", *args, ptr(dsum), ptr(count), ptr(dz),
         ptr(dbias if slab is None else None), int(accumulate), ptr(slab), ptr(ws), nb, dtype_code(z.dtype), _stream(z))
    if slab is not None:
        defer.append((lambda: slab_sum(slab, rows, C, C, dbias, accumulate), (slab,)))
    return dz


def gemm(a, b, trans_a=False, trans_b=False, bias=None, relu=False, out=None, out_dtype=torch.float32,
         accumulate=False, alpha=1.0, M=None, N=None, K=None, lda=None, ldb=None, ldc=None,
         batch=1, stride_a=0, stride_b=0, stride_c=0, splits=1):
    for t in (a, b, bias, out):
        if t is not None and not t.is_cuda:
            raise ValueError("libocrk ops take device tensors (got a CPU tensor)")
    if M is None:
        _chk(a, b)
        M, K = (a.shape[1], a.shape[0]) if trans_a else (a.shape[0], a.shape[1])
        N = b.shape[0] if trans_b else b.shape[1]
        lda, ldb = a.shape[1], b.shape[1]
    if out is None:
        out = torch.empty(M, N, dtype=out_dtype, device=a.device)
        ldc = N
    ldc = ldc if ldc is not None else N
    if a.dtype != b.dtype:
        raise TypeError("gemm operands must share a dtype")
    kc = -(-(-(-K // splits)) // 32) * 32 if splits > 1 else K
    splits = -(-K // kc) if splits > 1 else 1
    nb = _lib.lib().ocrk_gemm_workspace_size(M, N, batch, splits) if splits > 1 else 0
    ws = _ws(nb, a.device) if nb else None
    call("ocrk_gemm", int(trans_a), int(trans_b), M, N, K, float(alpha), ptr(a), lda, stride_a, ptr(b), ldb,
         stride_b, ptr(out), ldc, stride_c, dtype_code(out.dtype), ptr(bias), int(relu), int(accumulate),
         batch, dtype_code(a.dtype), splits, ptr(ws), nb, _stream(a))
    return out


_PERSISTENT = {}
# ... 450 lines not shown
```

### cnn_lstm_ctc_ocr_amd/model.py

```python
import contextlib

import numpy as np
import torch
import torch.distributed as dist

from . import kernels as K
from . import options
from .config import BN_EPS, BN_MOMENTUM, INFER, LAYER_PARAMS, POOLS, TRAIN, ModelConfig, rnn_size
from .params import ParamStore

layer_params = LAYER_PARAMS

_DEFAULT = []


@contextlib.contextmanager
def use_store(store):
    _DEFAULT.append(store)
    try:
        yield store
    finally:
        _DEFAULT.pop()


# ... 44 lines not shown
            ctx.conv12_bwd = bool(options.get("CONV12_BWD") and K.conv12_bwd_ok(x, dt))
            w_nk2, _ = store.conv_images(even, dt)
            y_odd, bits, z12, st12 = K.conv12_fwd(x, P["convnet/conv1/kernel"], P["convnet/conv1/bias"], w_nk2,
                                                  P[pe + "/bias"], want_y1=not ctx.conv12_bwd)
            ctx.relu_bits = bits if ctx.conv12_bwd or K.conv2_bwd_data_conv1_wgrad_ok(z12, x) else None
            zs = (z12, st12)
        elif k == 1 and training and dt == torch.bfloat16 and not ctx.exact and options.get("CONV1_FUSED"):
            y_odd, bits = K.conv1_fwd(x, P["convnet/conv1/kernel"], P["convnet/conv1/bias"], dt, relu_bits=True)
            ctx.relu_bits = bits if K.conv2_bwd_data_conv1_wgrad_ok(y_odd, x) else None
        elif k == 1:
            y_odd = K.conv1_fwd(x, P["convnet/conv1/kernel"], P["convnet/conv1/bias"], dt)
        else:
            w_nk, _ = store.conv_images(odd, dt)
            if (training and dt == torch.bfloat16 and not ctx.exact and options.get("RELU_BITS")
                    and K.relu_bits_ok(x.shape, x.shape[3], w_nk.shape[0], store.conv_images(even, dt)[0].shape[0],
                                       dt)):
                y_odd, ctx.relu_bits = K.conv3x3_fwd_relu_bits(x, w_nk, P[f"convnet/{odd}/bias"])
            else:
                y_odd = K.conv3x3_fwd(x, w_nk, P[f"convnet/{odd}/bias"], relu=True)
        B, H, W, _ = (y_odd if zs is None else zs[0]).shape
        M = B * H * W
        w_nk, _ = store.conv_images(even, dt)
        C = w_nk.shape[0]
        if training:
            if zs is not None:
                z, stats = zs
                trows = W
            elif K.conv3x3_fwd_rowstats_ok(y_odd, C):
                z, stats = K.conv3x3_fwd_rowstats(y_odd, w_nk, P[pe + "/bias"])
                trows = W
            else:
                stats = torch.empty(K.conv_stats_tiles(M), 2, C, dtype=torch.float32, device=x.device)
                z = K.conv3x3_fwd(y_odd, w_nk, P[pe + "/bias"], relu=False, stats=stats)
                trows = 128
            group = _bn_group(store)
            if group is not None:
                mean, invstd, count = K.bn_finalize_sync(stats, M, C, BN_EPS, BN_MOMENTUM,
                                                         store.stats[pe + "/batch_norm/moving_mean"],
                                                         store.stats[pe + "/batch_norm/moving_variance"], trows,
                                                         group)
                ctx.bn_sync = (group, count)
            else:
                mean, invstd = K.bn_finalize(stats, M, C, BN_EPS, BN_MOMENTUM,
                                             store.stats[pe + "/batch_norm/moving_mean"],
                                             store.stats[pe + "/batch_norm/moving_variance"], tile_rows=trows)
        else:
            z = K.conv3x3_fwd(y_odd, w_nk, P[pe + "/bias"], relu=False)
            mean, invstd = K.bn_infer_params(store.stats[pe + "/batch_norm/moving_mean"],
                                             store.stats[pe + "/batch_norm/moving_variance"], BN_EPS)
        p = K.bn_relu_pool_fwd(z, mean, invstd, P[pe + "/batch_norm/gamma"], P[pe + "/batch_norm/beta"],
                               POOLS[even], time_major=(k == 4))
        ctx.store, ctx.k = store, k
        ctx.save_for_backward(x, y_odd, z, mean, invstd, p)
        return p

    @staticmethod
    def backward(ctx, dp):
        with _conv_precision(ctx.exact):
            return _ConvBlock._backward(ctx, dp)

    @staticmethod
    def _backward(ctx, dp):
        store, k = ctx.store, ctx.k
        x, y_odd, z, mean, invstd, pooled = ctx.saved_tensors
        dt = store.cfg.dtype
        P, G = store.params, store.grads
        odd, even = f"conv{2 * k - 1}", f"conv{2 * k}"
        pe, po = f"convnet/{even}", f"convnet/{odd}"
        dp = dp.contiguous()
        if dp.dtype != dt:
            dp = K.cast(dp, dt)
        dz = K.bn_relu_pool_bwd(z, dp, mean, invstd, P[pe + "/batch_norm/gamma"], P[pe + "/batch_norm/beta"],
                                POOLS[even], dp_time_major=(k == 4),
                                dgamma=G[pe + "/batch_norm/gamma"], dbeta=G[pe + "/batch_norm/beta"],
                                dbias=G[pe + "/bias"],
                                sync=ctx.bn_sync,
                                pooled=pooled if ctx.bn_sync is None and ctx.pooled_bn else None)
        B, H, W, C = dz.shape
        if k > 1:
            with _conv_side(store, y_odd, dz, *_conv_late_tensors(store)):
                _conv_late_run(store)
                _conv_wgrad(ctx.exact, y_odd, dz, G[pe + "/kernel"])
        _, w_bwd = store.conv_images(even, dt)
        if ctx.conv12_bwd:
            if store.conv_late:
                with _conv_side(store, *_conv_late_tensors(store)):
                    _conv_late_run(store)
            K.conv12_bwd(dz, w_bwd, x, P["convnet/conv1/kernel"], P["convnet/conv1/bias"], G[pe + "/kernel"],
                         G[po + "/kernel"], G[po + "/bias"], relu_bits=ctx.relu_bits)
            store.join()
            return (None, None, None, None) + (None,) * (len(ctx.needs_input_grad) - 4)
        if ctx.c1_fused and K.conv2_bwd_data_conv1_wgrad_ok(dz, x):
            with _conv_side(store, y_odd, dz, *_conv_late_tensors(store)):
                _conv_late_run(store)
                _conv_wgrad(ctx.exact, y_odd, dz, G[pe + "/kernel"])
            bits = ctx.relu_bits
            K.conv2_bwd_data_conv1_wgrad(dz, w_bwd, None if bits is not None else y_odd, x, G[po + "/kernel"],
                                         G[po + "/bias"], relu_bits=bits)
            store.join()
            return (None, None, None, None) + (None,) * (len(ctx.needs_input_grad) - 4)
        if k > 1 and ctx.relu_bits is not None:
            dy_odd = K.conv3x3_bwd_data(dz, w_bwd, dbias=G[po + "/bias"], relu_bits=ctx.relu_bits)
        else:
            dy_odd = K.conv3x3_bwd_data(dz, w_bwd, relu_mask=y_odd, dbias=G[po + "/bias"] if k > 1 else None)
        dx = None
        if k == 1:
            with _conv_side(store, x, dy_odd, *_conv_late_tensors(store)):
                _conv_late_run(store)
                K.conv1_bwd_weight(x, dy_odd, G[po + "/kernel"], G[po + "/bias"])
            _conv_wgrad(ctx.exact, y_odd, dz, G[pe + "/kernel"])
            store.join()
        else:
            if k > 2 and options.get("CONV_SIDE") and options.get("SIDE_STREAM"):
                store.conv_late.append((lambda x=x, d=dy_odd, dw=G[po + "/kernel"], ex=ctx.exact:
                                        _conv_wgrad(ex, x, d, dw), (x, dy_odd)))
            else:
                with _conv_side(store, x, dy_odd):
                    _conv_wgrad(ctx.exact, x, dy_odd, G[po + "/kernel"])
            if ctx.needs_input_grad[0]:
                _, w_bwd_odd = store.conv_images(odd, dt)
                dx = K.conv3x3_bwd_data(dy_odd, w_bwd_odd)
        return (dx, None, None, None) + (None,) * (len(ctx.needs_input_grad) - 4)


def _bn_group(store):
    g = store.bn_group
    if g is None or not (dist.is_available() and dist.is_initialized()):
        return None
    return g if dist.get_world_size(g) > 1 else None


def _block_variables(store, k):
    names = [f"convnet/conv{2 * k - 1}/kernel", f"convnet/conv{2 * k - 1}/bias",
             f"convnet/conv{2 * k}/kernel", f"convnet/conv{2 * k}/bias",
             f"convnet/conv{2 * k}/batch_norm/gamma", f"convnet/conv{2 * k}/batch_norm/beta"]
    return [store.params[n] for n in names]


def convnet_layers(inputs, widths, mode, store=None):
    store = store or default_store()
    training = mode == TRAIN
    x = inputs
    if x.dim() == 4:
        if x.shape[-1] != 1:
            raise ValueError("inputs must be [batch, 32, width, 1]")
        x = x[..., 0]
    x = x.contiguous()
    if x.dtype not in (torch.uint8, store.cfg.dtype):
        x = K.cast(x, store.cfg.dtype)
    track = torch.is_grad_enabled() and training
    h = x
    for k in (1, 2, 3, 4):
        variables = _block_variables(store, k) if track else []
        if track:
            for v in variables:
                v.requires_grad_(True)
        h = _ConvBlock.apply(h, store, k, training, *variables)
    if not isinstance(widths, torch.Tensor):
        widths = torch.as_tensor(np.asarray(widths), dtype=torch.int32)
    widths = widths.to(device=h.device, dtype=torch.int32)
    sequence_length = K.seq_len(widths)
    return h.transpose(0, 1), sequence_length


_SIDE_STREAMS = {}


def _new_side_stream(dev, lane):
    return torch.cuda.Stream(device=dev)


class side_work:

    def __init__(self, store, *tensors, lane="side"):
        self.store, self.tensors, self.lane = store, tensors, lane
# ... 47 lines not shown
        dt = store.cfg.dtype
        T, B, n_in = x.shape
        H = store.cfg.rnn_sizes[layer - 1]
        wxT, _wx, whT, _wh, bias = store.lstm_images(layer, dt)
        gx = K.gemm(x.view(T * B, n_in), wxT, trans_b=True, bias=bias, out_dtype=dt)
        out, hprev, cprev, acts = K.lstm_fwd(gx, whT, seq_len, T, B, H, dt, save=any(ctx.needs_input_grad))
        ctx.store, ctx.layer, ctx.H = store, layer, H
        ctx.save_for_backward(x, seq_len, hprev, cprev, acts)
        return out

    @staticmethod
    def backward(ctx, dout):
        store, layer, H = ctx.store, ctx.layer, ctx.H
        x, seq_len, hprev, cprev, acts = ctx.saved_tensors
        dt = store.cfg.dtype
        T, B, n_in = x.shape
        G4 = 4 * H
        dout = dout.contiguous()
        if dout.dtype != dt:
            dout = K.cast(dout, dt)
        _wxT, wx, _whT, wh, _bias = store.lstm_images(layer, dt)
        dG = K.lstm_bwd(wh, seq_len, dout, cprev, acts, T, B, H, dbias=store.flat_bias_pair_grad(layer))
        R = T * B
        dx = None
        pre = f"rnn/bdrnn{layer}"
        with side_work(store, x, hprev, dG):
            gf, gb = store.grads[f"{pre}/fw/lstm_cell/kernel"], store.grads[f"{pre}/bw/lstm_cell/kernel"]
            sk = gf.numel()
            if dt == torch.float32 and not K.f32_mode_exact():
                (xh, xl), (hh, hl), (gh, gl) = K.split_bf16(x), K.split_bf16(hprev), K.split_bf16(dG)
                passes = [(xh, hh, gh), (xh, hh, gl), (xl, hl, gh)]
            else:
                passes = [(x, hprev, dG)]
            if gb.data_ptr() == gf.data_ptr() + 4 * sk:
                for _xa, ha, ga in passes:
                    K.gemm(ha.view(R, 2 * H), ga.view(R, 2 * G4), trans_a=True, out=gf[n_in:], accumulate=True,
                           M=H, N=G4, K=R, lda=2 * H, ldb=2 * G4, ldc=G4, batch=2, stride_a=H, stride_b=G4,
                           stride_c=sk, splits=_splits(H, G4, R, batch=2, items=_tn_items(layer)))
                for xa, _ha, ga in passes:
                    K.gemm(xa, ga.view(R, 2 * G4), trans_a=True, out=gf, accumulate=True, M=n_in, N=G4, K=R,
                           lda=n_in, ldb=2 * G4, ldc=G4, batch=2, stride_a=0, stride_b=G4, stride_c=sk,
                           splits=_splits(n_in, G4, R, batch=2, items=_tn_items(layer)))
            else:
                for xa, ha, ga in passes:
                    dg = ga.view(R, 2 * G4)
                    for d, gk in enumerate((gf, gb)):
                        dgd = dg[:, d * G4:]
                        K.gemm(xa, dgd, trans_a=True, out=gk, accumulate=True, M=n_in, N=G4, K=R, lda=n_in,
                               ldb=2 * G4, ldc=G4, splits=_splits(n_in, G4, R, items=_tn_items(layer)))
                        K.gemm(ha.view(R, 2 * H)[:, d * H:], dgd, trans_a=True, out=gk[n_in:], accumulate=True,
                               M=H, N=G4, K=R, lda=2 * H, ldb=2 * G4, ldc=G4,
                               splits=_splits(H, G4, R, items=_tn_items(layer)))
        if ctx.needs_input_grad[0]:
            dx = K.gemm(dG.view(R, 2 * G4), wx, trans_b=True, out_dtype=dt).view(T, B, n_in)
        return (dx,) + (None,) * (len(ctx.needs_input_grad) - 1)


class _BiGRU(torch.autograd.Function):

    @staticmethod
    def forward(ctx, x, seq_len, store, layer, *variables):
        dt = store.cfg.dtype
        T, B, n_in = x.shape
        H = store.cfg.rnn_sizes[layer - 1]
        wxT, _wx, whgT, whcT, _whg, _whc, bias = store.gru_images(layer, dt)
        gx = K.gemm(x.view(T * B, n_in), wxT, trans_b=True, bias=bias, out_dtype=dt)
        out, hprev, rh, acts = K.gru_fwd(gx, whgT, whcT, seq_len, T, B, H, dt)
        ctx.store, ctx.layer, ctx.H = store, layer, H
        ctx.save_for_backward(x, seq_len, hprev, rh, acts)
        return out

    @staticmethod
    def backward(ctx, dout):
        store, layer, H = ctx.store, ctx.layer, ctx.H
        x, seq_len, hprev, rh, acts = ctx.saved_tensors
        dt = store.cfg.dtype
        T, B, n_in = x.shape
        G2, G3 = 2 * H, 3 * H
        dout = dout.contiguous()
        if dout.dtype != dt:
            dout = K.cast(dout, dt)
        _wxT, wx, _whgT, _whcT, whg, whc, _bias = store.gru_images(layer, dt)
        dG = K.gru_bwd(whg, whc, seq_len, dout, hprev, acts, T, B, H, dbias=store.gru_bias_cat_grad(layer))
        pre = f"rnn/bdrnn{layer}"
        R = T * B
        side = side_work(store, x, hprev, rh, dG)
        side.__enter__()
        gf, gb = store.grads[f"{pre}/fw/gru_cell/gates/kernel"], store.grads[f"{pre}/bw/gru_cell/gates/kernel"]
        cf, cb = store.grads[f"{pre}/fw/gru_cell/candidate/kernel"], store.grads[f"{pre}/bw/gru_cell/candidate/kernel"]
        sk = (gb.data_ptr() - gf.data_ptr()) // 4
        batched = sk > 0 and cb.data_ptr() - cf.data_ptr() == 4 * sk
        if batched:
            dg = dG.view(R, 2 * G3)
            hp, rhv = hprev.view(R, 2 * H), rh.view(R, 2 * H)
            K.gemm(x, dg, trans_a=True, out=gf, accumulate=True, M=n_in, N=G2, K=R, lda=n_in, ldb=2 * G3,
                   ldc=G2, batch=2, stride_a=0, stride_b=G3, stride_c=sk, splits=_splits(n_in, G2, R, batch=2, items=_tn_items(layer)))
            K.gemm(hp, dg, trans_a=True, out=gf[n_in:], accumulate=True, M=H, N=G2, K=R, lda=2 * H, ldb=2 * G3,
                   ldc=G2, batch=2, stride_a=H, stride_b=G3, stride_c=sk, splits=_splits(H, G2, R, batch=2, items=_tn_items(layer)))
            K.gemm(x, dg[:, G2:], trans_a=True, out=cf, accumulate=True, M=n_in, N=H, K=R, lda=n_in,
                   ldb=2 * G3, ldc=H, batch=2, stride_a=0, stride_b=G3, stride_c=sk,
                   splits=_splits(n_in, H, R, batch=2, items=_tn_items(layer)))
            K.gemm(rhv, dg[:, G2:], trans_a=True, out=cf[n_in:], accumulate=True, M=H, N=H, K=R, lda=2 * H,
                   ldb=2 * G3, ldc=H, batch=2, stride_a=H, stride_b=G3, stride_c=sk, splits=_splits(H, H, R, batch=2, items=_tn_items(layer)))
        for d, dn in enumerate(() if batched else ("fw", "bw")):
            gk = store.grads[f"{pre}/{dn}/gru_cell/gates/kernel"]
            ck = store.grads[f"{pre}/{dn}/gru_cell/candidate/kernel"]
            dgg = dG.view(R, 2 * G3)[:, d * G3:]
            dgc = dG.view(R, 2 * G3)[:, d * G3 + G2:]
            hp = hprev.view(R, 2 * H)[:, d * H:]
            rhd = rh.view(R, 2 * H)[:, d * H:]
            K.gemm(x, dgg, trans_a=True, out=gk, accumulate=True, M=n_in, N=G2, K=R, lda=n_in,
                   ldb=2 * G3, ldc=G2, splits=_splits(n_in, G2, R, items=_tn_items(layer)))
            K.gemm(hp, dgg, trans_a=True, out=gk[n_in:], accumulate=True, M=H, N=G2, K=R, lda=2 * H,
                   ldb=2 * G3, ldc=G2, splits=_splits(H, G2, R, items=_tn_items(layer)))
            K.gemm(x, dgc, trans_a=True, out=ck, accumulate=True, M=n_in, N=H, K=R, lda=n_in,
                   ldb=2 * G3, ldc=H, splits=_splits(n_in, H, R, items=_tn_items(layer)))
            K.gemm(rhd, dgc, trans_a=True, out=ck[n_in:], accumulate=True, M=H, N=H, K=R, lda=2 * H,
                   ldb=2 * G3, ldc=H, splits=_splits(H, H, R, items=_tn_items(layer)))
        side.__exit__(None, None, None)
        dx = None
        if ctx.needs_input_grad[0]:
            dx = K.gemm(dG.view(R, 2 * G3), wx, trans_b=True, out_dtype=dt).view(T, B, n_in)
        return (dx,) + (None,) * (len(ctx.needs_input_grad) - 1)




def _tn_items(layer):
    if layer == 1:
        return options.get("TN_ITEMS_L1")
    return options.get("TN_ITEMS")


def _splits(M, N, Kdim, batch=1, items=None):
    if M >= 256 and N >= 256:
        tiles = -(-M // 256) * -(-N // 256) * batch
        return int(max(1, min((items or options.get("TN_ITEMS")) // tiles, Kdim // 1024)))
    tiles = -(-M // 128) * -(-N // 128) * batch
    return int(max(1, min(-(-512 // tiles), Kdim // 2048)))


class _Logits(torch.autograd.Function):

    @staticmethod
    def forward(ctx, x, store, *variables):
        dt = store.cfg.dtype
        T, B, D = x.shape
        wT = store.logits_image_t(dt)
        logits = K.gemm(x.view(T * B, D), wT, trans_b=True, bias=store.params["rnn/logits/bias"], relu=True)
        logits = logits.view(T, B, -1)
        ctx.store = store
        ctx.save_for_backward(x, logits)
        return logits

    @staticmethod
    def backward(ctx, dlogits):
        store = ctx.store
        x, logits = ctx.saved_tensors
        dt = store.cfg.dtype
        T, B, D = x.shape
        C = logits.shape[-1]
        R = T * B
        dpre = K.relu_mask(dlogits.contiguous(), logits, dt)
        with side_work(store, x, dpre):
            split = dt == torch.float32 and not K.f32_mode_exact() and x.numel() % 8 == 0 and dpre.numel() % 8 == 0
            for xa, pa in (K.split_products(x, dpre) if split else [(x, dpre)]):
                K.gemm(xa, pa, trans_a=True, out=store.grads["rnn/logits/kernel"], accumulate=True,
                       M=D, N=C, K=R, lda=D, ldb=C, ldc=C, splits=_splits(D, C, R))
            K.colsum(dpre, R, C, store.grads["rnn/logits/bias"])
        dx = None
        if ctx.needs_input_grad[0]:
            dx = K.gemm(dpre.view(R, C), store.logits_image(dt), trans_b=True, out_dtype=dt).view(T, B, D)
        return (dx,) + (None,) * (len(ctx.needs_input_grad) - 1)


# ... 148 lines not shown
```

### cnn_lstm_ctc_ocr_amd/options.py

```python
import contextlib
import os

_HOST_DEFAULTS = {
    "LSTM_PERSISTENT": 1,
    "F32_TRAIN_EXACT": 0,
    "SIDE_STREAM": 1,
    "CONV_SIDE": 1,
    "CONV12_FUSED": 1,
    "RELU_BITS": 1,
    "POOLED_BN": 1,
    "CONV1_FUSED": 1,
    "CONV12_BWD": 1,
    "TN_ITEMS": 256,
    "TN_ITEMS_L1": 160,
}
KERNEL_OPTIONS = ("CONV_DIRECT", "CONV_ROWS", "CONV_ROWS_WIDE", "CONV_WGRAD_BLOCKS", "LSTM_SPIN_LIMIT",
                  "PERSIST_LATE", "LSTM_BWD_R16", "CTC_LDS",
                  "PP_PERSIST_NK", "NT_F32_EXACT", "NT_F32_MASK",
                  "NT_F32_X6", "BEAM_WAVE", "BN_BWD_BLOCKS", "BN_ROUTE", "BN_ROUTE_SEG", "BN_ROUTE_NCH", "CONV_TN_ITEMS", "CONV_TN4_ITEMS",
                  "CONV_WGRAD_CUS", "F32_MFMA", "GEMM_NT", "GEMM_NT_STAGED", "GEMM_PP", "GEMM_PPTN", "PP_MIN_N", "GEMM_TN",
                  "LSTM_DMA", "LSTM_BWD_DMA", "LSTM_FWD_R16", "NT_TAP_UNIFORM")


def _env_int(name, default):
    v = os.environ.get("OCRK_" + name)
    if v is None or v == "":
        return default
    try:
        return int(v)
    except ValueError:
        raise ValueError(f"OCRK_{name}={v!r}: an integer is expected") from None


_HOST = {k: _env_int(k, d) for k, d in _HOST_DEFAULTS.items()}


def get(name):
    if name in _HOST:
        return _HOST[name]
    if name in KERNEL_OPTIONS:
        import ctypes

        from . import _lib
        v = ctypes.c_int64()
        _lib.call("ocrk_get_option", name.encode(), ctypes.byref(v))
        return v.value
    raise KeyError(f"unknown option {name!r}")


def set(name, value):
    value = int(value)
    if name in _HOST:
        prev, _HOST[name] = _HOST[name], value
        return prev
    if name in KERNEL_OPTIONS:
        import ctypes

        from . import _lib
        prev = ctypes.c_int64()
        _lib.call("ocrk_set_option", name.encode(), value, ctypes.byref(prev))
        return prev.value
    raise KeyError(f"unknown option {name!r}")

# ... 12 lines not shown
```

### cnn_lstm_ctc_ocr_amd/params.py

```python

import numpy as np
import torch

from . import kernels as K
from .config import LAYER_PARAMS, ModelConfig

_ALIGN = 64


def param_shapes(cfg):
    out = []
    cin = 1
    for filters, k, _pad, name, bn in LAYER_PARAMS:
        out.append((f"convnet/{name}/kernel", (k, k, cin, filters), True))
        out.append((f"convnet/{name}/bias", (filters,), True))
        if bn:
            out.append((f"convnet/{name}/batch_norm/gamma", (filters,), True))
            out.append((f"convnet/{name}/batch_norm/beta", (filters,), True))
            out.append((f"convnet/{name}/batch_norm/moving_mean", (filters,), False))
            out.append((f"convnet/{name}/batch_norm/moving_variance", (filters,), False))
        cin = filters
    n_in = cin
    for li, H in enumerate(cfg.rnn_sizes, start=1):
        pre = f"rnn/bdrnn{li}"
# ... 39 lines not shown
        bad = np.abs(x) > 2
    return x * std


def reference_init(cfg, seed=0):
    rng = np.random.default_rng(seed)
    vals = {}
    shapes = {n: sh for n, sh, _t in param_shapes(cfg)}
    for name in creation_order(cfg):
        shape = shapes[name]
        leaf = name.rsplit("/", 1)[1]
        if name.startswith("convnet") and leaf == "kernel":
            v = _trunc_normal(rng, shape, np.sqrt(2.6 / (shape[0] * shape[1] * shape[2])))
        elif name == "rnn/logits/kernel":
            v = _trunc_normal(rng, shape, np.sqrt(2.6 / shape[0]))
        elif "gru_cell" in name or ("lstm_cell" in name and leaf == "kernel"):
            v = _trunc_normal(rng, shape, 0.01)
        elif leaf in ("gamma", "moving_variance"):
            v = np.ones(shape)
        else:
            v = np.zeros(shape)
        vals[name] = v.astype(np.float32)
    return vals


class ParamStore:
    def __init__(self, cfg=None, device="cuda", seed=0, values=None):
        self.cfg = cfg or ModelConfig()
        self.device = torch.device(device)
        self.spec = param_shapes(self.cfg)
        self.offsets = {}
        sizes = {True: 0, False: 0}
        for name, shape, tr in self.spec:
            n = int(np.prod(shape))
            self.offsets[name] = (tr, sizes[tr], shape)
            sizes[tr] += (n + _ALIGN - 1) // _ALIGN * _ALIGN
        self.n_trainable = sum(int(np.prod(s)) for _, s, tr in self.spec if tr)
        self.flat = torch.zeros(sizes[True], dtype=torch.float32, device=self.device)
        self.flat_grad = torch.zeros_like(self.flat)
        self.flat_stats = torch.zeros(max(sizes[False], _ALIGN), dtype=torch.float32, device=self.device)
        self.params, self.grads, self.stats = {}, {}, {}
        for name, shape, tr in self.spec:
            _, off, _ = self.offsets[name]
            n = int(np.prod(shape))
            if tr:
                self.params[name] = self.flat[off:off + n].view(shape)
                self.grads[name] = self.flat_grad[off:off + n].view(shape)
            else:
                self.stats[name] = self.flat_stats[off:off + n].view(shape)
        self.version = 0
        self._images = {}
        self.pending = []
        self.conv_late = []
        self.bn_group = None
        self.f32_conv_exact = False
        self.load_state_dict(values if values is not None else reference_init(self.cfg, seed))

    def state_dict(self):
        out = {k: v.detach().cpu().numpy().copy() for k, v in self.params.items()}
        out.update({k: v.detach().cpu().numpy().copy() for k, v in self.stats.items()})
        return out

    def load_state_dict(self, values):
        for name, _shape, _tr in self.spec:
            if name not in values:
                raise KeyError(f"missing variable {name}")
            dst = self.params.get(name, self.stats.get(name))
            src = torch.as_tensor(np.asarray(values[name], dtype=np.float32))
            if tuple(src.shape) != tuple(dst.shape):
                raise ValueError(f"{name}: shape {tuple(src.shape)} != {tuple(dst.shape)}")
            dst.copy_(src.to(self.device))
        self.bump()

    def save(self, path):
        np.savez(path, **{k.replace("/", "__"): v for k, v in self.state_dict().items()})

    def load(self, path):
        with np.load(path, allow_pickle=False) as z:
            self.load_state_dict({k.replace("__", "/"): z[k] for k in z.files})

    def zero_grad(self):
        self.join()
        self.flat_grad.zero_()

    def join(self):
        while self.conv_late:
            fn, _tensors = self.conv_late.pop(0)
            fn()
        if self.pending:
            cur = torch.cuda.current_stream(self.device)
            for ev in self.pending:
                K.wait_mark(cur, ev)
            self.pending.clear()

    def bump(self):
        self.version += 1
        self._images.clear()
        self._plan_fresh = False

    def images(self, key, builder):
        plan = self._plan_for(key)
        if plan is not None:
            if not self._plan_fresh:
                K.copy_batch(plan["table"], plan["njobs"], plan["tiles"], self.flat)
                self._plan_fresh = True
            return plan["images"][key]
# ... 198 lines not shown
```

### include/ocrk.h

```cpp
#ifndef OCRK_H_
#define OCRK_H_

#include <stddef.h>
#include <stdint.h>

#ifdef __cplusplus
extern "C" {
#endif

#define OCRK_ABI_VERSION 7

enum ocrk_status {
    OCRK_OK = 0,
    OCRK_ERR_INVALID_ARG = 1,
    OCRK_ERR_HIP = 2,
    OCRK_ERR_INFEASIBLE = 3
};

enum ocrk_dtype { OCRK_F32 = 0, OCRK_BF16 = 1 };

int ocrk_set_f32_gemm_mode(int mode);
int ocrk_f32_gemm_exact(void);

enum ocrk_device_status {
// ... 68 lines not shown
                     int cout, void* y, int y_dtype, int relu, float* stats, int dtype, void* stream);
size_t ocrk_conv3x3_bwd_data_workspace_size(int B, int H, int W, int cin);
int ocrk_conv3x3_bwd_data(const void* dy, int B, int H, int W, int cout, const void* w_bwd, int cin,
                          void* dx, const void* relu_mask, float* dbias, int accumulate, void* ws,
                          size_t ws_bytes, int dtype, void* stream);
int ocrk_conv3x3_fwd_relu_bits_supported(int B, int H, int W, int cin, int cout, int dtype);
int ocrk_conv3x3_fwd_relu_bits(const void* x, int B, int H, int W, int cin, const void* w_nk, const float* bias,
                               int cout, void* y, void* relu_bits, int dtype, void* stream);
int ocrk_conv3x3_bwd_data_bits_supported(int B, int H, int W, int cout, int cin, int dtype);
int ocrk_conv3x3_bwd_data_bits(const void* dy, int B, int H, int W, int cout, const void* w_bwd, int cin,
                               void* dx, const void* relu_bits, float* dbias, int accumulate, void* ws,
                               size_t ws_bytes, int dtype, void* stream);
int ocrk_conv3x3_bwd_data_bits_slab(const void* dy, int B, int H, int W, int cout, const void* w_bwd, int cin,
                                    void* dx, const void* relu_bits, float* slab, int dtype, void* stream);
int ocrk_conv3x3_bwd_data_slab(const void* dy, int B, int H, int W, int cout, const void* w_bwd, int cin,
                               void* dx, const void* relu_mask, float* slab, int dtype, void* stream);
size_t ocrk_conv3x3_wgrad_workspace_size(int B, int H, int W, int cin, int cout);
int ocrk_conv3x3_bwd_weight(const void* x, const void* dy, int B, int H, int W, int cin, int cout,
                            float* dw, int accumulate, void* ws, size_t ws_bytes, int dtype, void* stream);

size_t ocrk_bn_finalize_workspace_size(int tiles, int C);
int ocrk_bn_finalize_tiles(const float* stats, int tiles, int tile_rows, int64_t M, int C, float eps,
                           float momentum, float* mean, float* invstd, float* moving_mean, float* moving_var,
                           void* ws, size_t ws_bytes, void* stream);
int ocrk_bn_finalize(const float* stats, int tiles, int64_t M, int C, float eps, float momentum,
                     float* mean, float* invstd, float* moving_mean, float* moving_var, void* ws, size_t ws_bytes,
                     void* stream);
int ocrk_bn_moments(const float* stats, int tiles, int tile_rows, int64_t M, int C, double* moments, void* ws,
                    size_t ws_bytes, void* stream);
int ocrk_bn_finalize_moments(const double* moments, int C, float eps, float momentum, float* mean, float* invstd,
                             float* moving_mean, float* moving_var, void* stream);
int ocrk_bn_infer_params(const float* moving_mean, const float* moving_var, int C, float eps,
                         float* mean, float* invstd, void* stream);
int ocrk_bn_relu_pool_fwd(const void* z, int B, int H, int W, int C, const float* mean,
                          const float* invstd, const float* gamma, const float* beta, int kh, int kw,
                          int sh, int sw, void* out, int time_major, int dtype, void* stream);
size_t ocrk_bn_bwd_workspace_size(int B, int H, int W, int C);
int ocrk_bn_relu_pool_bwd(const void* z, const void* dp, int B, int H, int W, int C, const float* mean,
                          const float* invstd, const float* gamma, const float* beta, int kh, int kw,
                          int sh, int sw, int dp_time_major, void* dz, float* dgamma, float* dbeta,
                          float* dbias, int accumulate, void* ws, size_t ws_bytes, int dtype, void* stream);
size_t ocrk_bn_bwd_bias_slab_rows(int B, int H, int W, int C, int kh, int kw, int sh, int sw);
int ocrk_bn_relu_pool_bwd_slab(const void* z, const void* dp, int B, int H, int W, int C, const float* mean,
                               const float* invstd, const float* gamma, const float* beta, int kh, int kw,
                               int sh, int sw, int dp_time_major, void* dz, float* dgamma, float* dbeta,
                               int accumulate, float* bias_slab, void* ws, size_t ws_bytes, int dtype,
                               void* stream);
size_t ocrk_bn_bwd_pooled_bias_slab_rows(int B, int H, int W, int C, int kh, int kw, int sh, int sw);
int ocrk_bn_relu_pool_bwd_pooled(const void* z, const void* pooled, const void* dp, int B, int H, int W, int C,
                                 const float* mean, const float* invstd, const float* gamma, const float* beta,
                                 int kh, int kw, int sh, int sw, int dp_time_major, void* dz, float* dgamma,
                                 float* dbeta, float* dbias, int accumulate, float* bias_slab, void* ws,
                                 size_t ws_bytes, int dtype, void* stream);
int ocrk_bn_relu_pool_bwd_reduce(const void* z, const void* dp, int B, int H, int W, int C, const float* mean,
                                 const float* invstd, const float* gamma, const float* beta, int kh, int kw,
                                 int sh, int sw, int dp_time_major, float* dgamma, float* dbeta, int accumulate,
                                 float* dsum, void* ws, size_t ws_bytes, int dtype, void* stream);
int ocrk_bn_relu_pool_bwd_apply(const void* z, const void* dp, int B, int H, int W, int C, const float* mean,
                                const float* invstd, const float* gamma, const float* beta, int kh, int kw,
                                int sh, int sw, int dp_time_major, const float* dsum, const double* count,
                                void* dz, float* dbias, int accumulate, float* bias_slab, void* ws,
                                size_t ws_bytes, int dtype, void* stream);

int ocrk_lstm_fwd_step(const void* gx, const void* whT, const void* h_in, void* h_out, float* c_state,
                       const int* seq_len, int s, int T, int B, int H, void* out, void* hprev_t,
                       float* cprev_t, void* acts_t, int dtype, void* stream);
int ocrk_lstm_bwd_step(const void* wh, const void* dg_in, void* dg_out, float* dc_state, const int* seq_len,
                       int s, int T, int B, int H, const void* dout, const float* cprev_t,
                       const void* acts_t, void* dG_t, int dtype, void* stream);
int ocrk_lstm_fwd_persistent_supported(int B, int H);
size_t ocrk_lstm_fwd_persistent_workspace_size(int B, int H);
int ocrk_lstm_fwd_persistent(const void* gx, const void* whT, const int* seq_len, int T, int B, int H,
                             void* out, void* hprev_t, float* cprev_t, void* acts_t, unsigned* err,
                             unsigned* flags, void* ws, size_t ws_bytes, void* stream);
int ocrk_lstm_fwd_persistent_f32_supported(int B, int H);
size_t ocrk_lstm_fwd_persistent_f32_workspace_size(int B, int H);
size_t ocrk_lstm_fwd_persistent_f32_flags_size(int B, int H);
int ocrk_lstm_fwd_persistent_f32(const float* gx, const float* whT, const int* seq_len, int T, int B, int H,
                                 float* out, float* hprev_t, float* cprev_t, float* acts_t, unsigned* err,
                                 unsigned* flags, void* ws, size_t ws_bytes, void* stream);
int ocrk_lstm_bwd_persistent_f32_supported(int B, int H);
size_t ocrk_lstm_bwd_persistent_f32_workspace_size(int B, int H);
int ocrk_lstm_bwd_persistent_f32(const float* wh, const int* seq_len, int T, int B, int H, const float* dout,
                                 const float* cprev_t, const float* acts_t, float* dG_t, unsigned* err,
                                 unsigned* flags, float* dbias_part, void* ws, size_t ws_bytes, void* stream);
int ocrk_lstm_bwd_persistent_supported(int B, int H);
int ocrk_lstm_bwd_persistent_slices(int B, int H);
size_t ocrk_lstm_bwd_persistent_workspace_size(int B, int H);
int ocrk_lstm_bwd_persistent(const void* wh, const int* seq_len, int T, int B, int H, const void* dout,
                             const float* cprev_t, const void* acts_t, void* dG_t, unsigned* err,
                             unsigned* flags, float* dbias_part, void* ws, size_t ws_bytes, void* stream);
int ocrk_gru_fwd_step(const void* gx, const void* whgT, const void* whcT, void* h, void* rh,
                      const int* seq_len, int s, int T, int B, int H, void* out, void* hprev_t, void* rh_t,
                      void* acts_t, int dtype, void* stream);
int ocrk_gru_fwd(const void* gx, const void* whgT, const void* whcT, void* h, void* rh, const int* seq_len,
                 int T, int B, int H, void* out, void* hprev_t, void* rh_t, void* acts_t, int dtype,
                 void* stream);
int ocrk_gru_bwd(const void* whg, const void* whc, void* dzg, void* dzc, float* dh_tot, float* direct,
                 const int* seq_len, int T, int B, int H, const void* dout, const void* hprev_t,
                 const void* acts_t, void* dG_t, int dtype, void* stream);
int ocrk_gru_fwd_persistent_supported(int B, int H);
size_t ocrk_gru_fwd_persistent_workspace_size(int B, int H);
int ocrk_gru_fwd_persistent(const void* gx, const void* whgT, const void* whcT, const int* seq_len, int T, int B,
                            int H, void* out, void* hprev_t, void* rh_t, void* acts_t, unsigned* err,
                            unsigned* flags, void* ws, size_t ws_bytes, void* stream);
int ocrk_gru_bwd_persistent_supported(int B, int H);
// ... 54 lines not shown
```

Measured before the change: 53260.

## Fuse pooled batch-norm backward sums into the upstream dgrad GEMM epilogues

Adds a BNS epilogue to the NT GEMM engine. The conv3x3 data-grad and LSTM/GRU input-grad GEMMs that produce the gradient of a pooled BN output now also accumulate that BN's backward reduction sums into a slab. The following BN backward then consumes the slab, so the separate sums pass no longer re-reads the pooled activations and the gradient. A fix-up kernel recomputes only the channel groups whose beta/gamma condition requires the z-based path. The trade-off is a heavier GEMM epilogue, more tiles routed to the NT engine, and extra bookkeeping to match tensors between forward and backward.

```diff
diff --git a/cnn_lstm_ctc_ocr_amd/_lib.py b/cnn_lstm_ctc_ocr_amd/_lib.py
--- a/cnn_lstm_ctc_ocr_amd/_lib.py
+++ b/cnn_lstm_ctc_ocr_amd/_lib.py
@@ -81,6 +81,16 @@
     "ocrk_bn_bwd_pooled_bias_slab_rows": [_i32, _i32, _i32, _i32, _i32, _i32, _i32, _i32],
     "ocrk_bn_relu_pool_bwd_pooled": [_p, _p, _p, _i32, _i32, _i32, _i32, _p, _p, _p, _p, _i32, _i32, _i32, _i32,
                                      _i32, _p, _p, _p, _p, _i32, _p, _p, _sz, _i32, _p],
+    "ocrk_bn_bwd_sums_slab_rows": [_i64],
+    "ocrk_conv3x3_bwd_data_bn_sums_supported": [_i32, _i32, _i32, _i32, _i32, _i32],
+    "ocrk_conv3x3_bwd_data_bn_sums": [_p, _i32, _i32, _i32, _i32, _p, _i32, _p, _p, _p, _p, _p, _i32, _p],
+    "ocrk_gemm_nt_bn_sums_supported": [_i32, _i32, _i32, _i64, _i64, _i32],
+    "ocrk_gemm_nt_bn_sums": [_i32, _i32, _i32, _p, _i64, _p, _i64, _p, _p, _p, _p, _p, _i32, _p],
+    "ocrk_bn_bwd_pooled_sums_rows": [_i32, _i32, _i32, _i32, _i32, _i32, _i32, _i32],
+    "ocrk_bn_bwd_pooled_sums": [_p, _p, _p, _i32, _i32, _i32, _i32, _p, _p, _p, _p, _i32, _i32, _i32, _i32,
+                                _i32, _p, _i32, _p, _sz, _i32, _p],
+    "ocrk_bn_relu_pool_bwd_sums": [_p, _p, _p, _i32, _i32, _i32, _i32, _p, _p, _p, _p, _i32, _i32, _i32, _i32,
+                                   _i32, _p, _p, _p, _p, _p, _i32, _p, _p, _sz, _i32, _p],
     "ocrk_bn_relu_pool_bwd_reduce": [_p, _p, _i32, _i32, _i32, _i32, _p, _p, _p, _p, _i32, _i32, _i32, _i32,
                                      _i32, _p, _p, _i32, _p, _p, _sz, _i32, _p],
     "ocrk_bn_relu_pool_bwd_apply": [_p, _p, _i32, _i32, _i32, _i32, _p, _p, _p, _p, _i32, _i32, _i32, _i32,
@@ -142,6 +152,8 @@
 _RESTYPE["ocrk_persistent_flags_size"] = ctypes.c_size_t
 _RESTYPE["ocrk_bn_bwd_bias_slab_rows"] = ctypes.c_size_t
 _RESTYPE["ocrk_bn_bwd_pooled_bias_slab_rows"] = ctypes.c_size_t
+_RESTYPE["ocrk_bn_bwd_sums_slab_rows"] = ctypes.c_size_t
+_RESTYPE["ocrk_bn_bwd_pooled_sums_rows"] = ctypes.c_size_t
 _RESTYPE["ocrk_crc32c"] = ctypes.c_uint32
 
 
diff --git a/cnn_lstm_ctc_ocr_amd/csrc/bn.hip b/cnn_lstm_ctc_ocr_amd/csrc/bn.hip
--- a/cnn_lstm_ctc_ocr_amd/csrc/bn.hip
+++ b/cnn_lstm_ctc_ocr_amd/csrc/bn.hip
@@ -493,7 +493,7 @@
 }
 
 
-template <typename T>
+template <typename T, bool FIXUP = false>
 __global__ void __launch_bounds__(256)
 bn_bwd_pooled_sums_kernel(const T* __restrict__ p, const T* __restrict__ dp, int64_t items, int C,
                           const float* __restrict__ gamma, const float* __restrict__ beta,
@@ -513,6 +513,11 @@
         rg[i] = ga != 0.f ? 1.f / ga : 0.f;
         bt[i] = be;
         s1[i] = s2[i] = 0.f;
+    }
+    __shared__ int zgroup[256];
+    if constexpr (FIXUP) {
+        if (!__syncthreads_or(from_z)) return;
+        if (threadIdx.x < G) zgroup[threadIdx.x] = from_z;
     }
     const int64_t i0 = (int64_t)blockIdx.x * items_per_block;
     const int64_t i1 = min(items, i0 + items_per_block);
@@ -560,7 +565,7 @@
                 s2[i] += d * ((zb[i] - mu[i]) * is[i]);
             }
         }
-    } else {
+    } else if constexpr (!FIXUP) {
         constexpr int U = 4;
         for (int64_t it = i0 + threadIdx.x; it < i1; it += 256 * U) {
             Pend8<T> pr[U], dr[U];
@@ -588,6 +593,9 @@
     __syncthreads();
     for (int o = threadIdx.x; o < 2 * C; o += 256) {
         const int which = o / C, c = o % C, gg = c / 8, ci = c % 8;
+        if constexpr (FIXUP) {
+            if (!zgroup[gg]) continue;
+        }
         float s = 0.f;
         for (int q = gg; q < 256; q += G) s += red[q][which * 8 + ci];
         slab[(int64_t)blockIdx.x * 2 * C + o] = s;
@@ -815,7 +823,7 @@
                        int dp_time_major, void* dz, float* dgamma, float* dbeta, float* dbias, int accumulate,
                        float* bias_slab_out, void* ws, size_t ws_bytes, int dtype, void* stream, int phase = 0,
                        float* dsum_out = nullptr, const float* dsum_in = nullptr, const double* count = nullptr,
-                       const void* pooled = nullptr) {
+                       const void* pooled = nullptr, float* sums_slab = nullptr, int sums_only = 0) {
     OCRK_REQUIRE(C % 8 == 0 && 256 % (C / 8) == 0, "ocrk_bn_relu_pool_bwd: C=%d unsupported", C);
     OCRK_REQUIRE(ws_bytes >= ocrk_bn_bwd_workspace_size(B, H, W, C), "ocrk_bn_relu_pool_bwd: workspace too small");
     const int64_t items = (int64_t)B * H * W * (C / 8);
@@ -845,7 +853,20 @@
         nr = (int)ocrk::cdiv(tasks, ocrk::cdiv(ocrk::cdiv(tasks, nbr), 256) * 256);
     }
     int st = OCRK_OK;
-    if (phase == 2) {
+    if (sums_slab && sums_only == 1) {
+        OCRK_REQUIRE(from_pooled && phase == 0, "ocrk_bn_bwd_pooled_sums: the pooled form is off for this pool");
+        slab = sums_slab;
+    }
+    if (sums_slab && sums_only != 1) {
+        OCRK_REQUIRE(from_pooled && phase == 0 && dtype == OCRK_BF16 && C % 16 == 0,
+                     "ocrk_bn_relu_pool_bwd_sums: needs the pooled form (a window-walk pool), bf16, C %% 16 == 0");
+        slab = sums_slab;
+        nr = (int)ocrk::cdiv(pitems / (C / 8), 128);
+        bn_bwd_pooled_sums_kernel<bf16, true><<<nr, 256, 0, s>>>((const bf16*)pooled, (const bf16*)dp, pitems, C, gamma,
+                                                                 beta, mean, invstd, (const bf16*)z, B, H, W, kh, kw,
+                                                                 sh, sw, dp_time_major, 128 * (C / 8), slab);
+        if (sums_only) return ocrk::launch_status("ocrk_bn_bwd_pooled_sums fix-up");
+    } else if (phase == 2) {
         bn_dsum_scale_kernel<<<ocrk::cdiv(2 * C, 256), 256, 0, s>>>(dsum_in, count, npix, 2 * C, dsum);
         st = ocrk::launch_status("ocrk_bn_relu_pool_bwd_apply scale");
         if (st) return st;
@@ -860,6 +881,7 @@
             bn_bwd_pooled_sums_kernel<float><<<nr, 256, 0, s>>>((const float*)pooled, (const float*)dp, pitems, C,
                                                                 gamma, beta, mean, invstd, (const float*)z, B, H, W,
                                                                 kh, kw, sh, sw, dp_time_major, ipb2, slab);
+        if (sums_only) return ocrk::launch_status("ocrk_bn_bwd_pooled_sums");
     } else if (rk) {
         const int Ho = (H - kh) / kh + 1, Wo = (W - kw) / sw + 1;
         const int nseg = (int)ocrk::cdiv(Wo, seg);
@@ -964,6 +986,45 @@
                        nullptr, nullptr, nullptr, pooled);
 }
 
+extern "C" size_t ocrk_bn_bwd_sums_slab_rows(int64_t pooled_pixels) {
+    return (size_t)std::max<int64_t>(1, ocrk::cdiv(pooled_pixels, 128));
+}
+
+extern "C" size_t ocrk_bn_bwd_pooled_sums_rows(int B, int H, int W, int C, int kh, int kw, int sh, int sw) {
+    if (C < 8 || C % 8 != 0 || H < kh || W < kw || !bn_route_variant(kh, kw, sh, sw, H, W)) return 0;
+    const int64_t items = (int64_t)B * H * W * (C / 8);
+    int64_t nb = bn_bwd_blocks(items);
+    nb = ocrk::cdiv(items, bn_bwd_ipb(items, nb));
+    const int64_t pitems = (int64_t)B * ((H - kh) / sh + 1) * ((W - kw) / sw + 1) * (C / 8);
+    const int64_t nr = std::max<int64_t>(1, std::min<int64_t>(nb, ocrk::cdiv(pitems, 256 * 4)));
+    return (size_t)ocrk::cdiv(pitems, ocrk::cdiv(ocrk::cdiv(pitems, nr), 256) * 256);
+}
+
+extern "C" int ocrk_bn_bwd_pooled_sums(const void* z, const void* pooled, const void* dp, int B, int H, int W, int C,
+                                       const float* mean, const float* invstd, const float* gamma, const float* beta,
+                                       int kh, int kw, int sh, int sw, int dp_time_major, float* sums_slab, int fixup,
+                                       void* ws, size_t ws_bytes, int dtype, void* stream) {
+    OCRK_REQUIRE(pooled && sums_slab, "ocrk_bn_bwd_pooled_sums: pooled and sums_slab are required");
+    return bn_bwd_impl(z, dp, B, H, W, C, mean, invstd, gamma, beta, kh, kw, sh, sw, dp_time_major, nullptr, nullptr,
+                       nullptr, nullptr, 0, nullptr, ws, ws_bytes, dtype, stream, 0, nullptr, nullptr, nullptr, pooled,
+                       sums_slab, fixup ? 2 : 1);
+}
+
+extern "C" int ocrk_bn_relu_pool_bwd_sums(const void* z, const void* pooled, const void* dp, int B, int H, int W,
+                                          int C, const float* mean, const float* invstd, const float* gamma,
+                                          const float* beta, int kh, int kw, int sh, int sw, int dp_time_major,
+                                          float* sums_slab, void* dz, float* dgamma, float* dbeta, float* dbias,
+                                          int accumulate, float* bias_slab, void* ws, size_t ws_bytes, int dtype,
+                                          void* stream) {
+    OCRK_REQUIRE(pooled && sums_slab, "ocrk_bn_relu_pool_bwd_sums: pooled and sums_slab are required");
+    OCRK_REQUIRE(bn_route_variant(kh, kw, sh, sw, H, W),
+                 "ocrk_bn_relu_pool_bwd_sums: the pooled form is off for this pool "
+                 "(ocrk_bn_bwd_pooled_bias_slab_rows() == 0)");
+    return bn_bwd_impl(z, dp, B, H, W, C, mean, invstd, gamma, beta, kh, kw, sh, sw, dp_time_major, dz, dgamma,
+                       dbeta, bias_slab ? nullptr : dbias, accumulate, bias_slab, ws, ws_bytes, dtype, stream, 0,
+                       nullptr, nullptr, nullptr, pooled, sums_slab);
+}
+
 extern "C" int ocrk_bn_relu_pool_bwd_reduce(const void* z, const void* dp, int B, int H, int W, int C,
                                             const float* mean, const float* invstd, const float* gamma,
                                             const float* beta, int kh, int kw, int sh, int sw, int dp_time_major,
diff --git a/cnn_lstm_ctc_ocr_amd/csrc/conv.hip b/cnn_lstm_ctc_ocr_amd/csrc/conv.hip
--- a/cnn_lstm_ctc_ocr_amd/csrc/conv.hip
+++ b/cnn_lstm_ctc_ocr_amd/csrc/conv.hip
@@ -267,6 +267,7 @@
                     void* y, int relu, float* stats, hipStream_t s);
 int conv_direct_bwd_data(const void* dy, int B, int H, int W, int cout, const void* w_bwd, int cin, void* dx,
                          const void* relu_mask, float* stats, hipStream_t s);
+bool conv_direct_bwd_data_covers(int B, int H, int W, int cout, int cin);
 size_t conv_direct_wgrad_ws_bytes(int B, int H, int W, int cin, int cout);
 int conv_direct_wgrad(const void* x, const void* dy, int B, int H, int W, int cin, int cout, float* dw,
                       int accumulate, void* ws, size_t ws_bytes, hipStream_t s);
@@ -539,6 +540,35 @@
     return bwd_data_run(dy, B, H, W, cout, w_bwd, cin, dx, relu_mask, slab, dtype, ocrk::as_stream(stream));
 }
 
+static ocrk::GemmParams bwd_data_bn_params(int B, int H, int W, int cout, int cin) {
+    ocrk::GemmParams p = {};
+    p.M = B * H * W; p.N = cin; p.K = 9 * cout; p.batch = 1;
+    p.ldb = 9 * cout; p.ldc = cin; p.c_bf16 = 1; p.alpha = 1.f;
+    p.splits = 1; p.k_chunk = (int)ocrk::cdiv(p.K, 32) * 32;
+    p.convH = H; p.convW = W; p.convC = cout;
+    return p;
+}
+
+extern "C" int ocrk_conv3x3_bwd_data_bn_sums_supported(int B, int H, int W, int cout, int cin, int dtype) {
+    if (dtype != OCRK_BF16 || B < 1 || H < 1 || W < 1 || (int64_t)B * H * W >= (1ll << 31)) return 0;
+    if (cin % 8 != 0 || cout % 8 != 0) return 0;
+    if (ocrk::conv_rows_dgrad_bits_covers(B, H, W, cin, cout) || ocrk::conv_direct_bwd_data_covers(B, H, W, cout, cin))
+        return 0;
+    return ocrk::gemm_nt_bn_sums_covers(bwd_data_bn_params(B, H, W, cout, cin), ocrk::A_IM2COL_FLIP) ? 1 : 0;
+}
+
+extern "C" int ocrk_conv3x3_bwd_data_bn_sums(const void* dy, int B, int H, int W, int cout, const void* w_bwd, int cin,
+                                             void* dx, const void* pooled, const float* gamma, const float* beta,
+                                             float* sums_slab, int dtype, void* stream) {
+    OCRK_REQUIRE(pooled && gamma && beta && sums_slab, "ocrk_conv3x3_bwd_data_bn_sums: pooled, gamma, beta, sums_slab");
+    OCRK_REQUIRE(ocrk_conv3x3_bwd_data_bn_sums_supported(B, H, W, cout, cin, dtype),
+                 "ocrk_conv3x3_bwd_data_bn_sums: B=%d H=%d W=%d %d<-%d dtype=%d not covered", B, H, W, cin, cout, dtype);
+    ocrk::GemmParams p = bwd_data_bn_params(B, H, W, cout, cin);
+    p.A = dy; p.B = w_bwd; p.C = dx;
+    p.bn_p = pooled; p.bn_gamma = gamma; p.bn_beta = beta; p.bn_slab = sums_slab;
+    return ocrk::gemm(p, ocrk::A_IM2COL_FLIP, ocrk::B_NK, dtype, ocrk::as_stream(stream));
+}
+
 static int conv_tn_items() {
     const int64_t v = ocrk::opt(ocrk::OPT_CONV_TN_ITEMS);
     return v >= 16 ? (int)v : 192;
diff --git a/cnn_lstm_ctc_ocr_amd/csrc/conv_direct.hip b/cnn_lstm_ctc_ocr_amd/csrc/conv_direct.hip
--- a/cnn_lstm_ctc_ocr_amd/csrc/conv_direct.hip
+++ b/cnn_lstm_ctc_ocr_amd/csrc/conv_direct.hip
@@ -531,6 +531,13 @@
     return splitk_finish(p, s);
 }
 
+bool conv_direct_bwd_data_covers(int B, int H, int W, int cout, int cin) {
+    const int mode = conv_direct_mode();
+    if (mode == 0 || (int64_t)B * H * W * (cin > cout ? cin : cout) * 2 > 0x7fffffffLL) return false;
+    if (mode == 1 && cin != 32) return false;
+    return (cout == 32 && cin == 32) || (cout == 64 && cin == 32) || (cout == 64 && cin == 64);
+}
+
 int conv_direct_bwd_data(const void* dy, int B, int H, int W, int cout, const void* w_bwd, int cin, void* dx,
                          const void* relu_mask, float* stats, hipStream_t s) {
     const int mode = conv_direct_mode();
diff --git a/cnn_lstm_ctc_ocr_amd/csrc/gemm.h b/cnn_lstm_ctc_ocr_amd/csrc/gemm.h
--- a/cnn_lstm_ctc_ocr_amd/csrc/gemm.h
+++ b/cnn_lstm_ctc_ocr_amd/csrc/gemm.h
@@ -26,6 +26,10 @@
     int epi_staged;
     const void* mask_bits;
     void* relu_bits;
+    const void* bn_p;
+    const float* bn_gamma;
+    const float* bn_beta;
+    float* bn_slab;
 };
 
 struct TileIdx { int bm, bn; bool valid; };
@@ -46,6 +50,7 @@
 int splitk_finish(const GemmParams& p, hipStream_t stream);
 
 int gemm_nt(const GemmParams& p, int amode, int bmode, int dtype, hipStream_t stream);
+bool gemm_nt_bn_sums_covers(const GemmParams& p, int amode);
 bool f32_exact_mfma();
 
 int gemm_pp(const GemmParams& p, int amode, int bmode, int dtype, hipStream_t stream);
diff --git a/cnn_lstm_ctc_ocr_amd/csrc/gemm.hip b/cnn_lstm_ctc_ocr_amd/csrc/gemm.hip
--- a/cnn_lstm_ctc_ocr_amd/csrc/gemm.hip
+++ b/cnn_lstm_ctc_ocr_amd/csrc/gemm.hip
@@ -552,6 +552,12 @@
     if (p.mask_bits || p.relu_bits) {
         const int st = gemm_nt(p, amode, bmode, dtype, stream);
         OCRK_REQUIRE(st >= 0, "gemm: ReLU bit masks need the NT engine (bf16 C, staged epilogue) for this shape");
+        return st;
+    }
+    if (p.bn_slab) {
+        const int st = gemm_nt(p, amode, bmode, dtype, stream);
+        OCRK_REQUIRE(st >= 0, "gemm: the pooled-BN sums epilogue does not cover this call (M=%d N=%d K=%d)", p.M, p.N,
+                     p.K);
         return st;
     }
     int nt = gemm_pp(p, amode, bmode, dtype, stream);
@@ -603,3 +609,31 @@
     int bmode = trans_b ? ocrk::B_NK : ocrk::B_KN;
     return ocrk::gemm(p, amode, bmode, dtype, ocrk::as_stream(stream));
 }
+
+namespace ocrk { bool gemm_pp_enabled(); }
+
+static ocrk::GemmParams gemm_bn_params(int M, int N, int K, int64_t lda, int64_t ldb) {
+    ocrk::GemmParams p = {};
+    p.M = M; p.N = N; p.K = K; p.batch = 1;
+    p.lda = lda; p.ldb = ldb; p.ldc = N; p.c_bf16 = 1; p.alpha = 1.f;
+    p.splits = 1; p.k_chunk = (int)ocrk::cdiv(K < 32 ? 32 : K, 32) * 32;
+    return p;
+}
+
+extern "C" int ocrk_gemm_nt_bn_sums_supported(int M, int N, int K, int64_t lda, int64_t ldb, int dtype) {
+    if (dtype != OCRK_BF16 || M < 1 || N < 1 || K < 1 || K % 8 != 0) return 0;
+    if (ocrk::gemm_pp_enabled() && M >= 4096 && N >= ocrk::opt(ocrk::OPT_PP_MIN_N)) return 0;
+    return ocrk::gemm_nt_bn_sums_covers(gemm_bn_params(M, N, K, lda, ldb), ocrk::A_ROWK) ? 1 : 0;
+}
+
+extern "C" int ocrk_gemm_nt_bn_sums(int M, int N, int K, const void* A, int64_t lda, const void* B, int64_t ldb,
+                                    void* C, const void* pooled, const float* gamma, const float* beta,
+                                    float* sums_slab, int dtype, void* stream) {
+    OCRK_REQUIRE(pooled && gamma && beta && sums_slab, "ocrk_gemm_nt_bn_sums: pooled, gamma, beta, sums_slab");
+    OCRK_REQUIRE(ocrk_gemm_nt_bn_sums_supported(M, N, K, lda, ldb, dtype),
+                 "ocrk_gemm_nt_bn_sums: M=%d N=%d K=%d dtype=%d not covered", M, N, K, dtype);
+    ocrk::GemmParams p = gemm_bn_params(M, N, K, lda, ldb);
+    p.A = A; p.B = B; p.C = C;
+    p.bn_p = pooled; p.bn_gamma = gamma; p.bn_beta = beta; p.bn_slab = sums_slab;
+    return ocrk::gemm(p, ocrk::A_ROWK, ocrk::B_NK, dtype, ocrk::as_stream(stream));
+}
diff --git a/cnn_lstm_ctc_ocr_amd/csrc/gemm_nt.hip b/cnn_lstm_ctc_ocr_amd/csrc/gemm_nt.hip
--- a/cnn_lstm_ctc_ocr_amd/csrc/gemm_nt.hip
+++ b/cnn_lstm_ctc_ocr_amd/csrc/gemm_nt.hip
@@ -14,7 +14,7 @@
 }
 
 template <int BM, int BN, int BK, int S, int WAVES_M, int AM, int NW = 4, bool F32 = false, bool EXACT = false,
-          bool X6 = false, bool TU = false>
+          bool X6 = false, bool TU = false, bool BNS = false>
 __global__ void __launch_bounds__(NW * 64) gemm_nt_kernel(const GemmParams p) {
     constexpr bool ST = NW == 4;
     constexpr int WAVES_N = NW / WAVES_M;
@@ -295,6 +295,20 @@
     }
     __syncthreads();
 
+    constexpr int BNS_NQ = BNS ? BM * (BN / 8) / (NW * 64) : 1;
+    uint4 bn_pq[BNS_NQ];
+    if constexpr (BNS) {
+        static_assert(BM == 128 && !F32 && (NW * 64) % (BN / 8) == 0 && (BM * (BN / 8)) % (NW * 64) == 0, "BNS tile");
+        const bf16* bp = reinterpret_cast<const bf16*>(p.bn_p);
+#pragma unroll
+        for (int k = 0; k < BNS_NQ; ++k) {
+            const int q = tid + k * NW * 64;
+            const int r = q / (BN / 8), cc = q - r * (BN / 8);
+            const int row = m0 + r, col = n0 + 8 * cc;
+            bn_pq[k] = make_uint4(0u, 0u, 0u, 0u);
+            if (row < p.M && col < p.N) bn_pq[k] = *reinterpret_cast<const uint4*>(bp + (int64_t)row * p.N + col);
+        }
+    }
     const int row_base = m0 + wm * WM + (lane >> 4) * 4;
     const int col_base = n0 + wn * WN + (lane & 15);
     if (p.splits > 1) {
@@ -376,7 +390,54 @@
                 acc[i][j][r] = v;
             }
     }
-    if (staged) {
+    if constexpr (BNS) {
+        static_assert(TILE_FITS && (NW * 64 / CPT) * 2 * BN * 4 <= S * STAGE, "BNS: the tile and the sums fit LDS");
+        __syncthreads();
+        const int cc = tid % CPT, gq = tid / CPT;
+        float rg[8], bt[8], s1[8], s2[8];
+#pragma unroll
+        for (int i = 0; i < 8; ++i) {
+            const int col = n0 + 8 * cc + i;
+            const float ga = col < p.N ? p.bn_gamma[col] : 0.f;
+            rg[i] = ga != 0.f ? 1.f / ga : 0.f;
+            bt[i] = col < p.N ? p.bn_beta[col] : 0.f;
+            s1[i] = s2[i] = 0.f;
+        }
+#pragma unroll
+        for (int k = 0; k < BNS_NQ; ++k) {
+            const int r = gq + k * (NW * 64 / CPT);
+            const int row = m0 + r, col = n0 + 8 * cc;
+            if (row < p.M && col < p.N) {
+                const uint4 v = *reinterpret_cast<const uint4*>(tile + r * TP + cc * 16);
+                *reinterpret_cast<uint4*>(Cb + (int64_t)row * p.ldc + col) = v;
+                const unsigned dw[4] = {v.x, v.y, v.z, v.w};
+                const unsigned pw[4] = {bn_pq[k].x, bn_pq[k].y, bn_pq[k].z, bn_pq[k].w};
+#pragma unroll
+                for (int i = 0; i < 8; ++i) {
+                    const float pv = __uint_as_float(i & 1 ? pw[i >> 1] & 0xffff0000u : pw[i >> 1] << 16);
+                    const float dv = __uint_as_float(i & 1 ? dw[i >> 1] & 0xffff0000u : dw[i >> 1] << 16);
+                    const float d = pv > 0.f ? dv : 0.f;
+                    s1[i] += d;
+                    s2[i] += d * ((pv - bt[i]) * rg[i]);
+                }
+            }
+        }
+        __syncthreads();
+        float* red = reinterpret_cast<float*>(smem);
+#pragma unroll
+        for (int i = 0; i < 8; ++i) {
+            red[(gq * 2 + 0) * BN + 8 * cc + i] = s1[i];
+            red[(gq * 2 + 1) * BN + 8 * cc + i] = s2[i];
+        }
+        __syncthreads();
+        for (int o = tid; o < 2 * BN; o += NW * 64) {
+            const int which = o / BN, c = o - which * BN;
+            float s = 0.f;
+            for (int q = 0; q < NW * 64 / CPT; ++q) s += red[(q * 2 + which) * BN + c];
+            if (n0 + c < p.N) p.bn_slab[(int64_t)tix.bm * 2 * p.N + (int64_t)which * p.N + n0 + c] = s;
+        }
+        return;
+    } else if (staged) {
         __syncthreads();
         uint8_t* rbits = reinterpret_cast<uint8_t*>(p.relu_bits);
         for (int q = tid; q < BM * CPT; q += NW * 64) {
@@ -471,6 +532,19 @@
     dim3 grid(xcd_grid((int)cdiv(p.M, BM), (int)cdiv(p.N, BN)), 1u, (unsigned)(p.batch * p.splits));
     gemm_nt_kernel<BM, BN, BK, S, WAVES_M, AM, NW, F32, EXACT, X6, TU><<<grid, NW * 64, LDS, stream>>>(p);
     return launch_status("gemm_nt");
+}
+
+template <int BN, int BK, int S, int WAVES_M, int AM, bool TU>
+int launch_nt_bns(const GemmParams& p, hipStream_t stream) {
+    constexpr int LDS = S * (128 + BN) * BK * 2;
+    static DeviceOnce configured;
+    set_dyn_lds(configured,
+                reinterpret_cast<const void*>(
+                    &gemm_nt_kernel<128, BN, BK, S, WAVES_M, AM, 4, false, false, false, TU, true>),
+                LDS);
+    dim3 grid(xcd_grid((int)cdiv(p.M, 128), (int)cdiv(p.N, BN)), 1u, 1u);
+    gemm_nt_kernel<128, BN, BK, S, WAVES_M, AM, 4, false, false, false, TU, true><<<grid, 256, LDS, stream>>>(p);
+    return launch_status("gemm_nt (pooled-BN sums)");
 }
 
 template <int BK, int AM>
@@ -542,6 +616,21 @@
     return launch_nt<128, 128, 64, 2, 2, AM>(p, s);
 }
 
+template <int BN, int BK, int S, int WAVES_M, int AM>
+int launch_nt_bns_tu(const GemmParams& p, hipStream_t s) {
+    if constexpr (AM != A_ROWK) {
+        if (nt_tap_uniform<BK, AM>(p)) return launch_nt_bns<BN, BK, S, WAVES_M, AM, true>(p, s);
+    }
+    return launch_nt_bns<BN, BK, S, WAVES_M, AM, false>(p, s);
+}
+
+template <int AM>
+int dispatch_nt_bns(const GemmParams& p, hipStream_t s) {
+    if (p.N <= 32) return launch_nt_bns_tu<32, 32, 3, 4, AM>(p, s);
+    if (p.N <= 64) return launch_nt_bns_tu<64, 32, 3, 2, AM>(p, s);
+    return launch_nt_bns_tu<128, 64, 2, 2, AM>(p, s);
+}
+
 }
 
 bool gemm_nt_enabled() {
@@ -552,7 +641,7 @@
     return opt(OPT_GEMM_NT_STAGED) != 0;
 }
 
-int gemm_nt(const GemmParams& p0, int amode, int bmode, int dtype, hipStream_t stream) {
+static int gemm_nt_run(const GemmParams& p0, int amode, int bmode, int dtype, hipStream_t stream, bool probe) {
     if (!gemm_nt_enabled() || bmode != B_NK) return -1;
     if (dtype == OCRK_F32) {
         const bool exact = f32_exact_mfma();
@@ -582,6 +671,18 @@
                    (!p.mask || (p.ldmask % 8 == 0 && (uintptr_t)p.mask % 16 == 0));
     if (p.K % 8 != 0 || (p.k_chunk < 512 && p.N > 64)) return -1;
     if ((p.mask_bits || p.relu_bits) && (!p.epi_staged || p.batch != 1 || p.ldc != p.N)) return -1;
+    if (p.bn_slab) {
+        if (!p.epi_staged || p.batch != 1 || p.mask || p.mask_bits || p.relu_bits || p.stats || p.bias || p.relu ||
+            p.alpha != 1.f || !p.bn_p || !p.bn_gamma || !p.bn_beta || (uintptr_t)p.bn_p % 16 != 0)
+            return -1;
+        if (p.N % 16 != 0 || 256 % (p.N / 8) != 0 || (p.N > 64 && p.N <= 96) || (p.N >= 512 && p.M >= 16384)) return -1;
+        if (amode == A_ROWK) {
+            if (p.lda % 8 != 0 || p.ldb % 8 != 0) return -1;
+            return probe ? OCRK_OK : dispatch_nt_bns<A_ROWK>(p, stream);
+        }
+        if (amode == A_IM2COL_FLIP) return probe ? OCRK_OK : dispatch_nt_bns<A_IM2COL_FLIP>(p, stream);
+        return -1;
+    }
     if (amode == A_ROWK) {
         if (p.lda % 8 != 0 || p.ldb % 8 != 0) return -1;
         return dispatch_nt<A_ROWK>(p, stream);
@@ -591,4 +692,19 @@
     return -1;
 }
 
-}
+int gemm_nt(const GemmParams& p, int amode, int bmode, int dtype, hipStream_t stream) {
+    return gemm_nt_run(p, amode, bmode, dtype, stream, false);
+}
+
+bool gemm_nt_bn_sums_covers(const GemmParams& p0, int amode) {
+    GemmParams p = p0;
+    float one = 0.f;
+    void* aligned = reinterpret_cast<void*>((uintptr_t)64);
+    p.C = aligned;
+    p.bn_p = aligned;
+    p.bn_gamma = p.bn_beta = &one;
+    p.bn_slab = &one;
+    return gemm_nt_run(p, amode, B_NK, OCRK_BF16, nullptr, true) == OCRK_OK;
+}
+
+}
diff --git a/cnn_lstm_ctc_ocr_amd/kernels.py b/cnn_lstm_ctc_ocr_amd/kernels.py
--- a/cnn_lstm_ctc_ocr_amd/kernels.py
+++ b/cnn_lstm_ctc_ocr_amd/kernels.py
@@ -219,6 +219,58 @@
     return dx
 
 
+class BnSums:
+
+    def __init__(self, pooled, gamma, beta):
+        self.pooled, self.gamma, self.beta = pooled, gamma, beta
+        self.slab = self.dp = None
+
+    def _new_slab(self, rows_of_dp, C):
+        rows = _lib.lib().ocrk_bn_bwd_sums_slab_rows(rows_of_dp)
+        return torch.empty(rows, 2 * C, dtype=torch.float32, device=self.pooled.device)
+
+
+def conv3x3_bwd_data_bn_sums_ok(dy, cin):
+    if dy.dtype != torch.bfloat16 or not dy.is_cuda:
+        return False
+    B, H, W, cout = dy.shape
+    return bool(_lib.lib().ocrk_conv3x3_bwd_data_bn_sums_supported(B, H, W, cout, cin, BF16))
+
+
+def conv3x3_bwd_data_bn_sums(dy, w_bwd, bn):
+    _chk(dy, w_bwd, bn.pooled, bn.gamma, bn.beta)
+    B, H, W, Cout = dy.shape
+    Cin = w_bwd.shape[0]
+    if bn.pooled.numel() != B * H * W * Cin or bn.pooled.dtype != dy.dtype:
+        raise ValueError("bn.pooled must have dx's size and dtype")
+    dx = torch.empty(B, H, W, Cin, dtype=dy.dtype, device=dy.device)
+    slab = bn._new_slab(B * H * W, Cin)
+    call("ocrk_conv3x3_bwd_data_bn_sums", ptr(dy), B, H, W, Cout, ptr(w_bwd), Cin, ptr(dx), ptr(bn.pooled),
+         ptr(bn.gamma), ptr(bn.beta), ptr(slab), dtype_code(dy.dtype), _stream(dy))
+    bn.slab, bn.dp = slab, dx
+    return dx
+
+
+def gemm_nt_bn_sums_ok(a, w_nk):
+    if a.dtype != torch.bfloat16 or w_nk.dtype != torch.bfloat16 or not a.is_cuda:
+        return False
+    (M, Kd), N = a.shape, w_nk.shape[0]
+    return bool(_lib.lib().ocrk_gemm_nt_bn_sums_supported(M, N, Kd, Kd, w_nk.shape[1], BF16))
+
+
+def gemm_nt_bn_sums(a, w_nk, bn):
+    _chk(a, w_nk, bn.pooled, bn.gamma, bn.beta)
+    (M, Kd), N = a.shape, w_nk.shape[0]
+    if bn.pooled.numel() != M * N or bn.pooled.dtype != a.dtype:
+        raise ValueError("bn.pooled must have the output's size and dtype")
+    out = torch.empty(M, N, dtype=a.dtype, device=a.device)
+    slab = bn._new_slab(M, N)
+    call("ocrk_gemm_nt_bn_sums", M, N, Kd, ptr(a), Kd, ptr(w_nk), w_nk.shape[1], ptr(out), ptr(bn.pooled),
+         ptr(bn.gamma), ptr(bn.beta), ptr(slab), dtype_code(a.dtype), _stream(a))
+    bn.slab, bn.dp = slab, out
+    return out
+
+
 def conv3x3_bwd_weight(x, dy, dw, accumulate=True):
     _chk(x, dy, dw)
     B, H, W, Cin = x.shape
@@ -298,8 +350,8 @@
 
 
 def bn_relu_pool_bwd(z, dp, mean, invstd, gamma, beta, pool, dp_time_major, dgamma, dbeta, accumulate=True,
-                     dbias=None, defer=None, sync=None, pooled=None):
-    _chk(z, dp, mean, invstd, gamma, beta, dgamma, dbeta, dbias, pooled)
+                     dbias=None, defer=None, sync=None, pooled=None, sums=None):
+    _chk(z, dp, mean, invstd, gamma, beta, dgamma, dbeta, dbias, pooled, sums)
     B, H, W, C = z.shape
     kh, kw, sh, sw = pool
     nb = _lib.lib().ocrk_bn_bwd_workspace_size(B, H, W, C)
@@ -318,9 +370,17 @@
         slab = None
         if dbias is not None and defer is not None:
             slab = torch.empty(rows, 2 * C, dtype=torch.float32, device=z.device)
-        call("ocrk_bn_relu_pool_bwd_pooled", ptr(z), ptr(pooled), ptr(dp), B, H, W, C, ptr(mean), ptr(invstd),
-             ptr(gamma), ptr(beta), kh, kw, sh, sw, int(dp_time_major), ptr(dz), ptr(dgamma), ptr(dbeta),
-             ptr(dbias), int(accumulate), ptr(slab), ptr(ws), nb, dtype_code(z.dtype), _stream(z))
+        if sums is not None:
+            srows = _lib.lib().ocrk_bn_bwd_sums_slab_rows(dp.numel() // C)
+            if sums.dtype != torch.float32 or sums.numel() != srows * 2 * C:
+                raise ValueError(f"sums must be f32 [{srows}, {2 * C}]")
+            call("ocrk_bn_relu_pool_bwd_sums", ptr(z), ptr(pooled), ptr(dp), B, H, W, C, ptr(mean), ptr(invstd),
+                 ptr(gamma), ptr(beta), kh, kw, sh, sw, int(dp_time_major), ptr(sums), ptr(dz), ptr(dgamma),
+                 ptr(dbeta), ptr(dbias), int(accumulate), ptr(slab), ptr(ws), nb, dtype_code(z.dtype), _stream(z))
+        else:
+            call("ocrk_bn_relu_pool_bwd_pooled", ptr(z), ptr(pooled), ptr(dp), B, H, W, C, ptr(mean), ptr(invstd),
+                 ptr(gamma), ptr(beta), kh, kw, sh, sw, int(dp_time_major), ptr(dz), ptr(dgamma), ptr(dbeta),
+                 ptr(dbias), int(accumulate), ptr(slab), ptr(ws), nb, dtype_code(z.dtype), _stream(z))
         if slab is not None:
             def _late():
                 slab_sum(slab, rows, C, 2 * C, dbias, accumulate)
@@ -340,6 +400,25 @@
          ptr(ws), nb,
          dtype_code(z.dtype), _stream(z))
     return dz
+
+
+def bn_bwd_pooled_sums(z, pooled, dp, mean, invstd, gamma, beta, pool, dp_time_major, slab=None):
+    _chk(z, pooled, dp, mean, invstd, gamma, beta, slab)
+    B, H, W, C = z.shape
+    kh, kw, sh, sw = pool
+    if slab is None:
+        rows = _lib.lib().ocrk_bn_bwd_pooled_sums_rows(B, H, W, C, kh, kw, sh, sw)
+        if rows == 0:
+            return None
+        out = torch.empty(rows, 2 * C, dtype=torch.float32, device=z.device)
+    else:
+        out = slab
+    nb = _lib.lib().ocrk_bn_bwd_workspace_size(B, H, W, C)
+    ws = _ws(nb, z.device)
+    call("ocrk_bn_bwd_pooled_sums", ptr(z), ptr(pooled), ptr(dp), B, H, W, C, ptr(mean), ptr(invstd), ptr(gamma),
+         ptr(beta), kh, kw, sh, sw, int(dp_time_major), ptr(out), int(slab is not None), ptr(ws), nb,
+         dtype_code(z.dtype), _stream(z))
+    return out
 
 
 def _bn_bwd_sync(z, dp, mean, invstd, gamma, beta, pool, dp_time_major, dgamma, dbeta, accumulate, dbias, defer,
diff --git a/cnn_lstm_ctc_ocr_amd/model.py b/cnn_lstm_ctc_ocr_amd/model.py
--- a/cnn_lstm_ctc_ocr_amd/model.py
+++ b/cnn_lstm_ctc_ocr_amd/model.py
@@ -120,6 +120,10 @@
                                POOLS[even], time_major=(k == 4))
         ctx.store, ctx.k = store, k
         ctx.save_for_backward(x, y_odd, z, mean, invstd, p)
+        store.bn_sums.pop(k, None)
+        if (training and dt == torch.bfloat16 and ctx.bn_sync is None and ctx.pooled_bn
+                and options.get("BN_FUSED_SUMS") and any(ctx.needs_input_grad)):
+            store.bn_sums[k] = K.BnSums(p, P[pe + "/batch_norm/gamma"], P[pe + "/batch_norm/beta"])
         return p
 
     @staticmethod
@@ -138,12 +142,14 @@
         dp = dp.contiguous()
         if dp.dtype != dt:
             dp = K.cast(dp, dt)
+        bn = store.bn_sums.pop(k, None)
+        sums = bn.slab if bn is not None and bn.dp is not None and _same_tensor(bn.dp, dp) else None
         dz = K.bn_relu_pool_bwd(z, dp, mean, invstd, P[pe + "/batch_norm/gamma"], P[pe + "/batch_norm/beta"],
                                 POOLS[even], dp_time_major=(k == 4),
                                 dgamma=G[pe + "/batch_norm/gamma"], dbeta=G[pe + "/batch_norm/beta"],
                                 dbias=G[pe + "/bias"],
                                 sync=ctx.bn_sync,
-                                pooled=pooled if ctx.bn_sync is None and ctx.pooled_bn else None)
+                                pooled=pooled if ctx.bn_sync is None and ctx.pooled_bn else None, sums=sums)
         B, H, W, C = dz.shape
         if k > 1:
             with _conv_side(store, y_odd, dz, *_conv_late_tensors(store)):
@@ -187,8 +193,30 @@
                     _conv_wgrad(ctx.exact, x, dy_odd, G[po + "/kernel"])
             if ctx.needs_input_grad[0]:
                 _, w_bwd_odd = store.conv_images(odd, dt)
-                dx = K.conv3x3_bwd_data(dy_odd, w_bwd_odd)
+                bn = _bn_sums_for(store, k - 1, x)
+                if bn is not None and K.conv3x3_bwd_data_bn_sums_ok(dy_odd, w_bwd_odd.shape[0]):
+                    dx = K.conv3x3_bwd_data_bn_sums(dy_odd, w_bwd_odd, bn)
+                else:
+                    dx = K.conv3x3_bwd_data(dy_odd, w_bwd_odd)
         return (dx, None, None, None) + (None,) * (len(ctx.needs_input_grad) - 4)
+
+
+def _same_tensor(a, b):
+    return a.data_ptr() == b.data_ptr() and a.numel() == b.numel() and a.dtype == b.dtype
+
+
+def _bn_sums_for(store, k, x):
+    bn = store.bn_sums.get(k)
+    if bn is None or not x.is_contiguous() or not _same_tensor(bn.pooled, x):
+        return None
+    return bn
+
+
+def _input_grad_gemm(store, layer, x, dg, wx):
+    bn = _bn_sums_for(store, 4, x) if layer == 1 else None
+    if bn is not None and dg.is_contiguous() and K.gemm_nt_bn_sums_ok(dg, wx):
+        return K.gemm_nt_bn_sums(dg, wx, bn)
+    return K.gemm(dg, wx, trans_b=True, out_dtype=x.dtype)
 
 
 def _bn_group(store):
@@ -342,7 +370,7 @@
                                M=H, N=G4, K=R, lda=2 * H, ldb=2 * G4, ldc=G4,
                                splits=_splits(H, G4, R, items=_tn_items(layer)))
         if ctx.needs_input_grad[0]:
-            dx = K.gemm(dG.view(R, 2 * G4), wx, trans_b=True, out_dtype=dt).view(T, B, n_in)
+            dx = _input_grad_gemm(store, layer, x, dG.view(R, 2 * G4), wx).view(T, B, n_in)
         return (dx,) + (None,) * (len(ctx.needs_input_grad) - 1)
 
 
@@ -410,7 +438,7 @@
         side.__exit__(None, None, None)
         dx = None
         if ctx.needs_input_grad[0]:
-            dx = K.gemm(dG.view(R, 2 * G3), wx, trans_b=True, out_dtype=dt).view(T, B, n_in)
+            dx = _input_grad_gemm(store, layer, x, dG.view(R, 2 * G3), wx).view(T, B, n_in)
         return (dx,) + (None,) * (len(ctx.needs_input_grad) - 1)
 
 
diff --git a/cnn_lstm_ctc_ocr_amd/options.py b/cnn_lstm_ctc_ocr_amd/options.py
--- a/cnn_lstm_ctc_ocr_amd/options.py
+++ b/cnn_lstm_ctc_ocr_amd/options.py
@@ -9,6 +9,7 @@
     "CONV12_FUSED": 1,
     "RELU_BITS": 1,
     "POOLED_BN": 1,
+    "BN_FUSED_SUMS": 1,
     "CONV1_FUSED": 1,
     "CONV12_BWD": 1,
     "TN_ITEMS": 256,
diff --git a/cnn_lstm_ctc_ocr_amd/params.py b/cnn_lstm_ctc_ocr_amd/params.py
--- a/cnn_lstm_ctc_ocr_amd/params.py
+++ b/cnn_lstm_ctc_ocr_amd/params.py
@@ -115,6 +115,7 @@
         self._images = {}
         self.pending = []
         self.conv_late = []
+        self.bn_sums = {}
         self.bn_group = None
         self.f32_conv_exact = False
         self.load_state_dict(values if values is not None else reference_init(self.cfg, seed))
diff --git a/include/ocrk.h b/include/ocrk.h
--- a/include/ocrk.h
+++ b/include/ocrk.h
@@ -144,6 +144,25 @@
                                  int kh, int kw, int sh, int sw, int dp_time_major, void* dz, float* dgamma,
                                  float* dbeta, float* dbias, int accumulate, float* bias_slab, void* ws,
                                  size_t ws_bytes, int dtype, void* stream);
+size_t ocrk_bn_bwd_sums_slab_rows(int64_t pooled_pixels);
+int ocrk_conv3x3_bwd_data_bn_sums_supported(int B, int H, int W, int cout, int cin, int dtype);
+int ocrk_conv3x3_bwd_data_bn_sums(const void* dy, int B, int H, int W, int cout, const void* w_bwd, int cin,
+                                  void* dx, const void* pooled, const float* gamma, const float* beta,
+                                  float* sums_slab, int dtype, void* stream);
+int ocrk_gemm_nt_bn_sums_supported(int M, int N, int K, int64_t lda, int64_t ldb, int dtype);
+int ocrk_gemm_nt_bn_sums(int M, int N, int K, const void* A, int64_t lda, const void* B, int64_t ldb, void* C,
+                         const void* pooled, const float* gamma, const float* beta, float* sums_slab, int dtype,
+                         void* stream);
+size_t ocrk_bn_bwd_pooled_sums_rows(int B, int H, int W, int C, int kh, int kw, int sh, int sw);
+int ocrk_bn_bwd_pooled_sums(const void* z, const void* pooled, const void* dp, int B, int H, int W, int C,
+                            const float* mean, const float* invstd, const float* gamma, const float* beta,
+                            int kh, int kw, int sh, int sw, int dp_time_major, float* sums_slab, int fixup,
+                            void* ws, size_t ws_bytes, int dtype, void* stream);
+int ocrk_bn_relu_pool_bwd_sums(const void* z, const void* pooled, const void* dp, int B, int H, int W, int C,
+                               const float* mean, const float* invstd, const float* gamma, const float* beta,
+                               int kh, int kw, int sh, int sw, int dp_time_major, float* sums_slab, void* dz,
+                               float* dgamma, float* dbeta, float* dbias, int accumulate, float* bias_slab,
+                               void* ws, size_t ws_bytes, int dtype, void* stream);
 int ocrk_bn_relu_pool_bwd_reduce(const void* z, const void* dp, int B, int H, int W, int C, const float* mean,
                                  const float* invstd, const float* gamma, const float* beta, int kh, int kw,
                                  int sh, int sw, int dp_time_major, float* dgamma, float* dbeta, int accumulate,
```

New measurement: 53370 (median of 6 runs). No clear change (+0.2%).
